# RHnejad/3D_PoseEstimation

Measured on AMD Instinct MI355X. Metric: poses/sec fwd+bwd, 17-joint lifting batch 4096; MPJPE vs ref, higher is better.
Workload: dtype f16x3 (two fp16 planes per fp32 operand, 3 fp16 MFMAs per product, fp32 accumulate); 1 GPU; BASELINE configs[1]: phase1_lifting LinearModel 34-1024-2x(1024-1024)-51, BN+ReLU+Dropout(0.5), one train_1.py step = zero_grad+forward+MSE+backward+AdamW; launch=eager (one call per kernel), per_gpu_batch=4096, global_batch=4096, parallelism=dp1

## Files before the change

### 3d_poseestimation_amd/_lib.py

```python
import ctypes
import os

import torch

_HERE = os.path.dirname(os.path.abspath(__file__))
LIB_PATH = os.environ.get("POSELIFT_LIB") or os.path.join(_HERE, "csrc", "libposelift.so")

PL_F32, PL_BF16, PL_BF16X6, PL_F16X3 = 0, 1, 2, 3


GATHER_FN = ctypes.CFUNCTYPE(ctypes.c_int, ctypes.c_void_p, ctypes.c_void_p, ctypes.c_int64, ctypes.c_void_p)


class PLSync(ctypes.Structure):
    _fields_ = [("world", ctypes.c_int32), ("rank", ctypes.c_int32), ("gather", GATHER_FN),
                ("user", ctypes.c_void_p)]


class PLL1Term(ctypes.Structure):
    _fields_ = [("a", ctypes.c_void_p), ("b", ctypes.c_void_p), ("n", ctypes.c_int64),
                ("da", ctypes.c_void_p), ("db", ctypes.c_void_p)]


L1_MAX_TERMS = 8


class PLDesc(ctypes.Structure):
    _fields_ = [
        ("in_dim", ctypes.c_int32), ("hidden", ctypes.c_int32), ("out_dim", ctypes.c_int32),
        ("num_stage", ctypes.c_int32), ("bn", ctypes.c_int32), ("dtype", ctypes.c_int32),
        ("p_dropout", ctypes.c_float), ("bn_eps", ctypes.c_float), ("bn_momentum", ctypes.c_float),
        ("reserved", ctypes.c_int32),
        ("params", ctypes.c_void_p), ("bn_running", ctypes.c_void_p), ("bn_batches", ctypes.c_void_p),
        ("sync", ctypes.POINTER(PLSync)),
        ("step_dev", ctypes.c_void_p),
        ("wplanes", ctypes.c_void_p), ("wplanes_valid", ctypes.c_int32), ("reserved2", ctypes.c_int32),
    ]


ADAMW_MAX_SEGS = 8


class PLAdamWSeg(ctypes.Structure):
    _fields_ = [("offset", ctypes.c_int64), ("numel", ctypes.c_int64), ("h", ctypes.c_void_p), ("l", ctypes.c_void_p)]


class PLAdamWPlanes(ctypes.Structure):
    _fields_ = [("nseg", ctypes.c_int32), ("kind", ctypes.c_int32), ("scale", ctypes.c_float),
                ("reserved", ctypes.c_int32), ("seg", PLAdamWSeg * ADAMW_MAX_SEGS)]


class PLAdamWStep(ctypes.Structure):
    _fields_ = [("m", ctypes.c_void_p), ("v", ctypes.c_void_p), ("lr", ctypes.c_float), ("lr_dev", ctypes.c_void_p),
                ("beta1", ctypes.c_float), ("beta2", ctypes.c_float), ("eps", ctypes.c_float), ("weight_decay", ctypes.c_float),
                ("t", ctypes.c_int64), ("t_dev", ctypes.c_void_p)]


class PLPlanesEpilogue(ctypes.Structure):
    _fields_ = [("bias", ctypes.c_void_p), ("scale", ctypes.c_void_p), ("shift", ctypes.c_void_p), ("resid", ctypes.c_void_p),
                ("relu", ctypes.c_int32), ("reserved", ctypes.c_int32), ("y_planes", ctypes.c_void_p)]


_c = ctypes
_P = ctypes.c_void_p
_D = ctypes.POINTER(PLDesc)
SIGNATURES = {
    "pl_version": (_c.c_int, []),
    "pl_last_error": (_c.c_char_p, []),
    "pl_num_hidden": (_c.c_int64, [_D]),
    "pl_param_tensors": (_c.c_int64, [_D]),
    "pl_param_offset": (_c.c_int64, [_D, _c.c_int64]),
    "pl_param_numel": (_c.c_int64, [_D, _c.c_int64]),
    "pl_param_arena_floats": (_c.c_int64, [_D]),
    "pl_workspace_bytes": (_c.c_size_t, [_D, _c.c_int64]),
    "pl_workspace_view": (_c.c_int, [_D, _c.c_int64, _c.c_int, _c.c_int64,
                                     _c.POINTER(_c.c_size_t), _c.POINTER(_c.c_size_t)]),
    "pl_workspace_bitmap_format": (_c.c_int, [_D, _c.c_int64, _c.c_int64]),
    "pl_lifter_fwd_eval": (_c.c_int, [_D, _P, _P, _c.c_int64, _P, _c.c_size_t, _P]),
    "pl_lifter_fwd_train": (_c.c_int, [_D, _P, _P, _c.c_int64, _P, _c.c_size_t, _c.c_uint64,
                                       _c.c_uint64, _P, _P]),
    "pl_lifter_bwd": (_c.c_int, [_D, _P, _P, _c.c_int64, _P, _c.c_size_t, _P, _P, _P]),
    "pl_lifter_fwd_eval_saved": (_c.c_int, [_D, _P, _P, _c.c_int64, _P, _c.c_size_t, _P]),
    "pl_lifter_bwd_eval": (_c.c_int, [_D, _P, _P, _c.c_int64, _P, _c.c_size_t, _P, _P, _P]),
    "pl_lifter_bwd_layers": (_c.c_int, [_D, _P, _P, _c.c_int64, _P, _c.c_size_t, _P, _P, _c.c_int, _c.c_int, _P]),
    "pl_lifter_train_fwd_bwd": (_c.c_int, [_D, _P, _P, _c.c_int64, _P, _c.c_size_t, _c.c_uint64, _c.c_uint64,
                                           _P, _P, _P, _c.c_int, _c.c_int, _P]),
    "pl_lifter_step_carries_adamw": (_c.c_int, [_D, _c.c_int64]),
    "pl_lifter_train_step": (_c.c_int, [_D, _P, _P, _c.c_int64, _P, _c.c_size_t, _c.c_uint64, _c.c_uint64,
                                        _P, _P, _P, _c.POINTER(PLAdamWStep), _P]),
    "pl_mse_scratch_bytes": (_c.c_size_t, [_c.c_int64]),
    "pl_mse_fwd_bwd": (_c.c_int, [_P, _P, _c.c_int64, _c.c_float, _P, _P, _P, _P]),
    "pl_l1_scratch_bytes": (_c.c_size_t, [_c.c_int]),
    "pl_l1_terms_fwd_bwd": (_c.c_int, [_c.POINTER(PLL1Term), _c.c_int, _c.c_float, _P, _P, _P]),
    "pl_mpjpe_scratch_bytes": (_c.c_size_t, [_c.c_int64, _c.c_int64]),
    "pl_mpjpe_accum": (_c.c_int, [_P, _P, _c.c_int64, _c.c_int64, _P, _P, _P]),
    "pl_adamw_flat": (_c.c_int, [_P, _P, _P, _P, _c.c_int64, _c.c_float, _c.c_float, _c.c_float,
                                 _c.c_float, _c.c_float, _c.c_int64, _c.c_float, _P]),
    "pl_adamw_flat_dev": (_c.c_int, [_P, _P, _P, _P, _c.c_int64, _P, _c.c_float, _c.c_float, _c.c_float,
                                     _c.c_float, _c.c_int64, _P, _c.c_float, _P]),
    "pl_adamw_flat_planes": (_c.c_int, [_P, _P, _P, _P, _c.c_int64, _c.c_float, _P, _c.c_float, _c.c_float, _c.c_float,
                                        _c.c_float, _c.c_int64, _P, _c.c_float, _c.POINTER(PLAdamWPlanes), _P]),
    "pl_wplanes_bytes": (_c.c_size_t, [_D]),
    "pl_wplanes_layer_bytes": (_c.c_size_t, [_D]),
    "pl_weight_plane_scale": (_c.c_float, []),
    "pl_wplanes_refresh": (_c.c_int, [_D, _P]),
    "pl_flip_pose": (_c.c_int, [_P, _P, _c.c_int64, _c.c_int64, _c.c_int64, _P]),
    "pl_counter_add": (_c.c_int, [_P, _c.c_int64, _P]),
    "pl_flip_pose_ex": (_c.c_int, [_P, _P, _P, _c.c_int64, _c.c_int64, _c.c_int64, _c.c_float, _c.c_float, _P]),
    "pl_flip_w_nhwc": (_c.c_int, [_P, _P, _c.c_int64, _c.c_int64, _c.c_int64, _c.c_int64, _P]),
    "pl_softargmax3d_nhwc_fwd": (_c.c_int, [_P, _c.c_int64, _c.c_int64, _c.c_int64, _c.c_int64, _P, _P, _P]),
    "pl_softargmax3d_nhwc_bwd": (_c.c_int, [_P, _P, _P, _c.c_int64, _c.c_int64, _c.c_int64, _c.c_int64, _P, _P]),
    "pl_conv2d_nhwc_scratch_bytes": (_c.c_size_t, [_c.c_int64, _c.c_int64, _c.c_int64, _c.c_int64, _c.c_int64,
                                                  _c.c_int, _c.c_int, _c.c_int, _c.c_int]),
    "pl_conv2d_nhwc_scratch_bytes_ex": (_c.c_size_t, [_c.c_int64, _c.c_int64, _c.c_int64, _c.c_int64, _c.c_int64,
                                                     _c.c_int, _c.c_int, _c.c_int, _c.c_int, _c.c_int, _c.c_int, _c.c_int]),
    "pl_conv2d_nhwc_fwd": (_c.c_int, [_P, _c.c_int64, _c.c_int64, _c.c_int64, _c.c_int64, _P, _c.c_int64, _c.c_int,
                                      _c.c_int, _c.c_int, _c.c_int, _P, _P, _P, _c.c_int, _P, _P, _c.c_int, _P, _c.c_size_t,
                                      _P]),
    "pl_conv2d_nhwc_wgrad_scratch_bytes": (_c.c_size_t, [_c.c_int64, _c.c_int64, _c.c_int64, _c.c_int64, _c.c_int64,
                                                        _c.c_int, _c.c_int, _c.c_int, _c.c_int]),
    "pl_conv2d_nhwc_wgrad": (_c.c_int, [_P, _c.c_int64, _c.c_int64, _c.c_int64, _c.c_int64, _P, _c.c_int64, _c.c_int,
                                        _c.c_int, _c.c_int, _c.c_int, _P, _c.c_int, _P, _c.c_size_t, _P]),
    "pl_bn_train_scratch_bytes": (_c.c_size_t, [_c.c_int64, _c.c_int64]),
    "pl_bn_train_fwd": (_c.c_int, [_P, _c.c_int64, _c.c_int64, _P, _P, _c.c_float, _c.c_float, _P, _P, _P, _c.c_int,
                                   _P, _P, _P, _P, _P, _P]),
    "pl_bn_train_bwd": (_c.c_int, [_P, _P, _P, _P, _P, _P, _c.c_int64, _c.c_int64, _P, _P, _P, _P, _P]),
    "pl_add_relu_fwd": (_c.c_int, [_P, _P, _c.c_int64, _c.c_int64, _P, _P, _P]),
    "pl_mask_by_bits": (_c.c_int, [_P, _P, _c.c_int64, _c.c_int64, _P, _P]),
    "pl_conv_act_plane_scale": (_c.c_float, []),
    "pl_planes_split": (_c.c_int, [_P, _c.c_int64, _c.c_int, _c.c_float, _P, _P]),
    "pl_planes_split_strided": (_c.c_int, [_P, _P, _P, _c.c_int, _c.c_float, _P, _P]),
    "pl_bn_train_fwd_ex": (_c.c_int, [_P, _c.c_int64, _c.c_int64, _P, _P, _c.c_float, _c.c_float, _P, _P, _P, _c.c_int,
                                      _P, _P, _P, _P, _P, _P, _c.c_int, _P, _P, _P]),
    "pl_gemm_stat_groups": (_c.c_int, [_c.c_int64]),
    "pl_bn_train_bwd_ex": (_c.c_int, [_P, _P, _P, _P, _P, _P, _c.c_int64, _c.c_int64, _P, _P, _P, _P, _P, _c.c_int, _P, _P]),
    "pl_add_relu_fwd_ex": (_c.c_int, [_P, _P, _c.c_int64, _c.c_int64, _P, _P, _P, _c.c_int, _P]),
    "pl_mask_add_by_bits": (_c.c_int, [_P, _P, _P, _c.c_int64, _c.c_int64, _P, _P]),
    "pl_bn_join_bwd": (_c.c_int, [_P, _P, _P, _P, _P, _P, _P, _c.c_int64, _c.c_int64, _P, _P, _P, _P, _P, _P, _c.c_int, _P, _P]),
    "pl_maxpool3x3s2_nhwc": (_c.c_int, [_P, _c.c_int64, _c.c_int64, _c.c_int64, _c.c_int64, _P, _P]),
    "pl_maxpool3x3s2_nhwc_bwd": (_c.c_int, [_P, _P, _c.c_int64, _c.c_int64, _c.c_int64, _c.c_int64, _P, _P]),
    "pl_maxpool3x3s2_nhwc_idx": (_c.c_int, [_P, _c.c_int64, _c.c_int64, _c.c_int64, _c.c_int64, _P, _P, _P]),
    "pl_maxpool3x3s2_nhwc_bwd_idx": (_c.c_int, [_P, _P, _c.c_int64, _c.c_int64, _c.c_int64, _c.c_int64, _P, _P]),
    "pl_upsample2x_zero_nhwc": (_c.c_int, [_P, _c.c_int64, _c.c_int64, _c.c_int64, _c.c_int64, _P, _P]),
    "pl_colsum_scratch_bytes": (_c.c_size_t, [_c.c_int64, _c.c_int64]),
    "pl_colsum": (_c.c_int, [_P, _c.c_int64, _c.c_int64, _P, _P, _P]),
    "pl_deconv4x4s2_nhwc_scratch_bytes": (_c.c_size_t, [_c.c_int64, _c.c_int64, _c.c_int64, _c.c_int64]),
    "pl_deconv4x4s2_nhwc_fwd": (_c.c_int, [_P, _c.c_int64, _c.c_int64, _c.c_int64, _c.c_int64, _P, _c.c_int64, _P, _P,
                                           _c.c_int, _P, _c.c_int, _P, _c.c_size_t, _P]),
    "pl_nhwc_to_nchw": (_c.c_int, [_P, _c.c_int64, _c.c_int64, _c.c_int64, _P, _P]),
    "pl_gather_rows2": (_c.c_int, [_P, _c.c_int64, _P, _c.c_int64, _P, _c.c_int64, _c.c_int64, _P, _P, _P]),
    "pl_flip_tta_pack": (_c.c_int, [_P, _P, _c.c_int64, _c.c_int64, _c.c_int64, _P]),
    "pl_flip_tta_merge": (_c.c_int, [_P, _P, _c.c_int64, _c.c_int64, _c.c_int64, _P]),
    "pl_softargmax_dl_scale": (_c.c_int, [_P, _c.c_int64, _c.c_int, _P, _P]),
    "pl_softargmax_fwd": (_c.c_int, [_P, _c.c_int64, _c.c_int64, _c.c_int64, _c.c_int64, _c.c_int, _c.c_int, _P, _P, _P]),
    "pl_softargmax_bwd": (_c.c_int, [_P, _P, _P, _c.c_int64, _c.c_int64, _c.c_int64, _c.c_int64, _c.c_int, _c.c_int,
                                     _P, _P]),
    "pl_gemm_f32": (_c.c_int, [_c.c_int, _P, _P, _P, _c.c_int64, _c.c_int64, _c.c_int64, _P,
                               _c.c_int, _P, _P]),
    "pl_gemm_arith": (_c.c_int, [_c.c_int, _c.c_int, _P, _P, _P, _c.c_int64, _c.c_int64, _c.c_int64, _P,
                                 _c.c_int, _P, _P]),
    "pl_gemm_planes_scratch_bytes": (_c.c_size_t, [_c.c_int64, _c.c_int64, _c.c_int64]),
    "pl_gemm_planes": (_c.c_int, [_c.c_int, _c.c_int, _P, _P, _P, _c.c_int64, _c.c_int64, _c.c_int64, _P,
                                  _c.c_float, _c.c_float, _P, _P]),
    "pl_gemm_planes_splits": (_c.c_int, [_c.c_int64, _c.c_int64, _c.c_int64]),
    "pl_gemm_planes_raw": (_c.c_int, [_c.c_int, _c.c_int, _P, _c.c_int64, _c.c_int64, _P, _c.c_int64, _c.c_int64, _P,
                                      _c.c_int64, _c.c_int64, _c.c_int64, _P, _c.c_float, _P, _P, _P, _P]),
    "pl_conv2d_planes_fwd": (_c.c_int, [_c.c_int, _P, _c.c_int64, _c.c_int64, _c.c_int64, _c.c_int64, _c.c_int64, _P,
                                        _c.c_int64, _c.c_int64, _c.c_int, _c.c_int, _c.c_int, _c.c_int, _P, _c.c_float, _P, _P, _P]),
    "pl_softargmax3d_nhwc_bwd_ex": (_c.c_int, [_P, _P, _P, _c.c_int64, _c.c_int64, _c.c_int64, _c.c_int64, _P, _P, _c.c_int,
                                               _P, _P]),
# ... 118 lines not shown
```

### 3d_poseestimation_amd/csrc/api.hip

```cpp
#include <stdarg.h>
#include <stdio.h>
#include <stdlib.h>

#include <vector>

#include "adamw.h"
#include "pl_internal.h"

namespace pl {

static thread_local char g_err[512] = "";

void set_error(const char* fmt, ...) {
  va_list ap;
  va_start(ap, fmt);
  vsnprintf(g_err, sizeof(g_err), fmt, ap);
  va_end(ap);
}

namespace {

inline int64_t align_up(int64_t v, int64_t a) { return (v + a - 1) / a * a; }

int check_desc(const PLDesc* d, bool need_arenas) {
// ... 47 lines not shown

struct ParamLayout {
  int L;
  std::vector<int64_t> off, numel;
  int64_t total;
};

ParamLayout param_layout(const PLDesc* d) {
  ParamLayout p;
  p.L = 1 + 2 * d->num_stage;
  int64_t o = 0;
  auto add = [&](int64_t n) {
    p.off.push_back(o);
    p.numel.push_back(n);
    o = align_up(o + n, 64);
  };
  for (int l = 0; l < p.L; ++l) {
    const int64_t fan_in = l == 0 ? d->in_dim : d->hidden;
    add((int64_t)d->hidden * fan_in);
    add(d->hidden);
    add(d->hidden);
    add(d->hidden);
  }
  add((int64_t)d->out_dim * d->hidden);
  add(d->out_dim);
  p.total = o;
  return p;
}

int out_splits(int M, int N, int K) {
  const int tiles = ((M + 127) / 128) * ((N + 127) / 128);
  int s = 256 / tiles;
  const int kmax = K / 128;
  if (s > kmax) s = kmax;
  return s < 1 ? 1 : s;
}

enum class Lin : uint8_t {
  Skinny, Planes, Gemm,
  PlanesMid,
  F32Mid,
};
enum class Stats : uint8_t {
  None,
  InLayer,
  Small,
  InApply,
  Finalize,
};
enum class Bwd : uint8_t {
  PlanesPair, F32Pair,
  SmallLayer, SmallLayerDw,
  InAbove,
  First,
};
struct LayerRoute {
  Lin lin;
  Stats stats;
  Bwd bwd;
  int groups;
  bool bnr_fused;
};
enum class Loss : uint8_t { SmallMse, FromSlabs, PartialOnly };

struct Ws {
  int L, G, RC;
  std::vector<size_t> z, act, bits, mean, rstd, dbpart;
  size_t stat, scale, shift, coef, ga, gb, dz, slabs, outpart, dyout, mse, total;
  size_t act_bytes, bits_bytes;
  size_t slab_floats;
  bool planes;
  int pkind;
  std::vector<size_t> actp, wp;
  std::vector<size_t> sactp;
  std::vector<char> act_f32;
  size_t dzp, amax, dzscale;
  size_t skp_out, skp_in;
  std::vector<size_t> wslab;
  std::vector<LayerRoute> layer;
  bool bn_small;
  bool small_layer;
  bool top_fused;
  bool adam_rides;
  bool small_f16;
  bool eval_small;
  bool out_narrow;
  bool out_skinny;
  Loss loss;
};

Ws plan(const PLDesc* d, int64_t B) {
  Ws w;
  w.L = 1 + 2 * d->num_stage;
  const int H = d->hidden;
  w.G = gemm_stat_groups((int)B);
  w.RC = bwd_row_chunks((int)B, H);
  size_t o = 0;
  auto take = [&](size_t bytes) {
    const size_t at = o;
    o = (size_t)align_up((int64_t)(o + bytes), 256);
    return at;
  };
  w.act_bytes = (size_t)B * H * sizeof(float);
  w.bits_bytes = std::max((size_t)B * bitmap_words_per_row(H), (size_t)H) * sizeof(uint64_t);
  w.pkind = planes_kind(d, B);
  w.planes = w.pkind != 0;
  for (int l = 0; l < w.L; ++l) {
    const bool f32 = !w.planes || (l % 2 == 0) || l == w.L - 1;
    w.act_f32.push_back(f32 ? 1 : 0);
    w.z.push_back(take(w.act_bytes));
    w.act.push_back(f32 ? take(w.act_bytes) : 0);
    w.bits.push_back(take(w.bits_bytes));
    w.mean.push_back(take((size_t)H * 4));
    w.rstd.push_back(take((size_t)H * 4));
    w.dbpart.push_back(take((size_t)w.RC * H * 4));
  }
  const int Pmax = std::max(std::max(w.G, skinny_stat_groups((int)B)), w.RC);
  const size_t amax_pairs = std::max((size_t)((H + 255) / 256) * w.RC, (size_t)(B / 64 + 1) * (H / 32 + 1));
  w.stat = take((size_t)sync_world(d) * ((size_t)2 * Pmax * H + 2 * amax_pairs) * 4);
  w.scale = take((size_t)w.L * H * 4);
  w.shift = take((size_t)w.L * H * 4);
  w.coef = take((size_t)3 * H * 4);
  w.ga = take(w.act_bytes);
  w.gb = take(w.act_bytes);
  w.dz = take(w.act_bytes);
  size_t slab = 0;
  auto need = [&](int M, int N) {
    const int s = tn_splits(M, N, (int)B);
    if (s > 1) slab = std::max(slab, (size_t)s * M * N * 4);
  };
  need(H, d->in_dim);
  need(H, H);
  need(d->out_dim, H);
  {
    const int so = out_splits((int)B, d->out_dim, H);
    if (so > 1) slab = std::max(slab, (size_t)so * B * d->out_dim * 4);
    slab = std::max(slab, (size_t)skinny_chunks((int)B) * std::max(d->in_dim, d->out_dim) * H * 4);
    slab = std::max(slab, skinny_narrow_out_part_floats((int)B, H) * 4);
    if (B <= kThinGemmMaxM && B % 128) slab = std::max(slab, thin_gemm_scratch_floats((int)B, H, H) * 4);
    if (B <= kThinGemmMaxM) slab = std::max(slab, (size_t)(H / 16 + 1) * B * 64 * 4);
  }
  w.slab_floats = slab / 4;
  w.slabs = take(slab);
  w.outpart = take((size_t)std::max(colsum_chunks((int)B), skinny_in_chunks((int)B)) * d->out_dim * 4);
  w.dyout = take((size_t)B * d->out_dim * 4);
  w.mse = take(std::max(pl_mse_scratch_bytes(B * d->out_dim), (size_t)256));
  w.dzp = w.amax = w.dzscale = 0;
  w.skp_out = take((size_t)skinny_in_chunks((int)B) * d->out_dim * H * 4);
  w.skp_in = take((size_t)skinny_in_chunks((int)B) * d->in_dim * H * 4);
  if (w.planes) {
    w.wslab.push_back(0);
    for (int l = 1; l < w.L; ++l) w.wslab.push_back(take((size_t)tn_splits(H, H, (int)B) * H * H * 4));
    for (int l = 0; l + 1 < w.L; ++l) w.actp.push_back(take(w.act_bytes));
    w.wp.push_back(0);
    for (int l = 1; l < w.L; ++l) w.wp.push_back(take((size_t)H * H * 4));
    w.dzp = take(w.act_bytes);
    w.amax = take(std::max((size_t)((H + 255) / 256) * w.RC, (size_t)(B / 64) * (H / 32)) * 2 * 4);
    w.dzscale = take((size_t)w.L * 2 * 4);
  }
  if (d->dtype == PL_F16X3 && B <= kThinGemmMaxM)
    for (int l = 0; l + 1 < w.L; ++l) w.sactp.push_back(take(w.act_bytes));
  w.total = o;

  const int world = sync_world(d);
  const bool first_ok = small_first_ok(d->in_dim), mid_ok = B * world <= 512 && small_layer_ok(2, H, H);
  w.bn_small = d->bn && !w.planes && world == 1 && B >= 2 && B <= kBnSmallRows;
  w.small_layer = w.bn_small && small_layer_ok((int)B, H, H);
  w.top_fused = w.small_layer && small_top_ok(d->out_dim);
  const bool small_head = w.top_fused && (d->num_stage > 0 || first_ok);
  w.adam_rides = small_head && H % 128 == 0;
  w.small_f16 = d->dtype == PL_F16X3 && !w.sactp.empty() && first_ok;
  w.eval_small = d->bn && B <= kThinGemmMaxM && small_layer_ok(2, H, H) && first_ok && small_top_ok(d->out_dim);
  w.out_narrow = skinny_narrow_out_supported(H, d->out_dim);
  w.out_skinny = skinny_supported(d->out_dim, H);
  const int so = w.out_narrow ? skinny_narrow_out_splits((int)B, H) : 0;
  w.loss = small_head ? Loss::SmallMse : (so && mse_from_slabs_supported(so, d->out_dim)) ? Loss::FromSlabs : Loss::PartialOnly;
  for (int l = 0; l < w.L; ++l) {
    LayerRoute r;
    if (l == 0) r.lin = skinny_supported(d->in_dim, H) ? Lin::Skinny : Lin::Gemm;
    else if (w.planes) r.lin = w.pkind == 2 && mid_ok ? Lin::PlanesMid : Lin::Planes;
    else r.lin = d->bn && d->dtype != PL_BF16 && B > kBnSmallRows && mid_ok ? Lin::F32Mid : Lin::Gemm;
    r.groups = r.lin == Lin::Skinny ? skinny_stat_groups((int)B) : w.G;
    const bool tile = w.small_layer && (l > 0 || first_ok);
    if (!d->bn) r.stats = Stats::None;
    else if (w.bn_small) r.stats = tile ? Stats::InLayer : Stats::Small;
    else r.stats = world == 1 && r.groups >= 1 && r.groups <= 4 ? Stats::InApply : Stats::Finalize;
    if (l == 0) r.bwd = tile && w.L > 1 ? Bwd::InAbove : Bwd::First;
    else if (!w.small_layer) r.bwd = w.planes ? Bwd::PlanesPair : Bwd::F32Pair;
    else r.bwd = H % 128 == 0 ? Bwd::SmallLayerDw : Bwd::SmallLayer;
    r.bnr_fused = w.planes && (l < w.L - 1 || w.out_skinny);
    w.layer.push_back(r);
  }
  return w;
}

struct BnrSlab {
  float *mine, *amax_mine, *amax0;
  int64_t floats_per_rank;
  int world;
};
BnrSlab bnr_slab(const PLDesc* d, const Ws& w, void* ws, int rc, int n_amax, bool eval_bn) {
  BnrSlab b;
  float* stat = reinterpret_cast<float*>(static_cast<char*>(ws) + w.stat);
  b.world = eval_bn ? 1 : sync_world(d);
  const int64_t sums = (int64_t)2 * rc * d->hidden;
  if (b.world == 1) {
    b.mine = stat;
    b.amax_mine = b.amax0 = w.amax ? reinterpret_cast<float*>(static_cast<char*>(ws) + w.amax) : nullptr;
    b.floats_per_rank = sums;
    return b;
  }
  b.floats_per_rank = sums + 2 * (int64_t)n_amax;
  b.mine = stat + (size_t)sync_rank(d) * b.floats_per_rank;
  b.amax_mine = b.mine + sums;
  b.amax0 = stat + sums;
  return b;
}

struct Layer {
  const float *W, *b, *gamma, *beta;
  float *gW, *gb, *ggamma, *gbeta;
  float *rm, *rv;
  int64_t* nbt;
  int K;
};

Layer layer_of(const PLDesc* d, const ParamLayout& pl_, float* grads, int l) {
  Layer y;
  const int H = d->hidden;
  y.K = l == 0 ? d->in_dim : H;
  y.W = d->params + pl_.off[4 * l];
  y.b = d->params + pl_.off[4 * l + 1];
  y.gamma = d->params + pl_.off[4 * l + 2];
  y.beta = d->params + pl_.off[4 * l + 3];
  y.gW = grads ? grads + pl_.off[4 * l] : nullptr;
  y.gb = grads ? grads + pl_.off[4 * l + 1] : nullptr;
  y.ggamma = grads ? grads + pl_.off[4 * l + 2] : nullptr;
  y.gbeta = grads ? grads + pl_.off[4 * l + 3] : nullptr;
  y.rm = d->bn_running ? d->bn_running + (size_t)l * 2 * H : nullptr;
  y.rv = d->bn_running ? d->bn_running + (size_t)l * 2 * H + H : nullptr;
  y.nbt = d->bn_batches ? d->bn_batches + l : nullptr;
  return y;
}

inline float* f32(void* ws, size_t off) { return reinterpret_cast<float*>(static_cast<char*>(ws) + off); }
inline uint64_t* u64(void* ws, size_t off) { return reinterpret_cast<uint64_t*>(static_cast<char*>(ws) + off); }

int check_ws(const Ws& w, void* ws, size_t bytes) {
  if (!ws) PL_FAIL(PL_EWORKSPACE, "workspace is NULL");
  if (reinterpret_cast<uintptr_t>(ws) & 255) PL_FAIL(PL_EWORKSPACE, "workspace not 256-byte aligned");
  if (bytes < w.total) PL_FAIL(PL_EWORKSPACE, "workspace too small: %zu < %zu bytes", bytes, w.total);
  return PL_OK;
}

inline unsigned short* u16(void* ws, size_t off) { return reinterpret_cast<unsigned short*>(static_cast<char*>(ws) + off); }
inline const unsigned short* sact_in(const Ws& w, void* ws, int l) { return w.small_f16 && l > 0 ? u16(ws, w.sactp[l - 1]) : nullptr; }
inline unsigned short* sact_out(const Ws& w, void* ws, int l) { return w.small_f16 && l + 1 < w.L ? u16(ws, w.sactp[l]) : nullptr; }

inline unsigned short* wplane(const PLDesc* d, const Ws& w, void* ws, int l) {
  if (d->wplanes) {
    const size_t per = (size_t)d->hidden * d->hidden * 2 * (w.pkind == 2 ? 2 : 1);
    return reinterpret_cast<unsigned short*>(static_cast<char*>(d->wplanes) + (size_t)(l - 1) * per);
  }
  return u16(ws, w.wp[l]);
}

int split_weight_planes(const PLDesc* d, const ParamLayout& P, const Ws& w, void* ws, hipStream_t s) {
  if (d->wplanes && d->wplanes_valid) return PL_OK;
  if (d->wplanes && (reinterpret_cast<uintptr_t>(d->wplanes) & 15)) PL_FAIL(PL_EINVAL, "wplanes not 16-byte aligned");
  const int64_t n = (int64_t)d->hidden * d->hidden;
  for (int l = 1; l < w.L; ++l) {
    unsigned short* q = wplane(d, w, ws, l);
    PlaneOut po = {q, q + n, kWeightPlaneScale, nullptr, w.pkind};
    PL_TRY(launch_split_planes(d->params + P.off[4 * l], n, po, s));
  }
  return PL_OK;
}

PlanesGemmArgs planes_args(int pkind, const unsigned short* A, int64_t a_plane, int lda, const unsigned short* Bm,
                           int64_t b_plane, int ldb, float* C, int M, int N, int K, float out_scale,
                           const float* dyn_inv) {
  PlanesGemmArgs g = {};
  g.A = A; g.B = Bm; g.a_plane = a_plane; g.b_plane = b_plane; g.lda = lda; g.ldb = ldb;
  g.mode = pkind == 2 ? 2 : 0;
  g.out_scale = pkind == 2 ? out_scale : 1.0f;
  g.dyn_inv = pkind == 2 ? dyn_inv : nullptr;
  g.e.C = C; g.e.M = M; g.e.N = N; g.e.K = K; g.e.ldc = N; g.e.split_k = 1;
  return g;
}

int gemm_out_layer(bool narrow, const float* h, const float* W, const float* bias, float* y, int M, int N, int K,
                   float* slabs, hipStream_t s) {
  if (narrow) return launch_skinny_narrow_out(h, W, bias, y, M, K, N, slabs, s);
  GemmArgs g = {};
  g.A = h; g.B = W; g.M = M; g.N = N; g.K = K; g.lda = K; g.ldb = K; g.ldc = N;
  const int splits = out_splits(M, N, K);
  if (splits > 1) {
    g.C = slabs; g.split_k = splits;
    PL_TRY(launch_gemm_f32(kNT, g, s));
    return launch_reduce_slabs_bias(slabs, splits, M, N, bias, y, s);
  }
  g.C = y; g.bias = bias; g.split_k = 1;
  return launch_gemm_f32(kNT, g, s);
}

int gemm_tn_reduced(const float* A, int lda, const float* Bm, int ldb, float* C, int M, int N, int K,
                    float* slabs, hipStream_t s) {
  GemmArgs g = {};
  g.A = A; g.B = Bm; g.M = M; g.N = N; g.K = K; g.lda = lda; g.ldb = ldb; g.ldc = N;
  const int splits = tn_splits(M, N, K);
  if (splits > 1) {
    g.C = slabs; g.split_k = splits;
    PL_TRY(launch_gemm_f32(kTN, g, s));
    return launch_reduce_slabs(slabs, splits, (int64_t)M * N, C, s);
  }
  g.C = C; g.split_k = 1;
  return launch_gemm_f32(kTN, g, s);
}

}
}

using namespace pl;

extern "C" int pl_version(void) { return PL_VERSION; }
extern "C" const char* pl_last_error(void) { return g_err; }

extern "C" int64_t pl_num_hidden(const PLDesc* d) { return d ? 1 + 2 * (int64_t)d->num_stage : PL_EINVAL; }
extern "C" int64_t pl_param_tensors(const PLDesc* d) { return d ? 4 * (1 + 2 * (int64_t)d->num_stage) + 2 : PL_EINVAL; }
extern "C" int64_t pl_param_offset(const PLDesc* d, int64_t i) {
  if (check_desc(d, false) != PL_OK) return PL_EINVAL;
  const ParamLayout p = param_layout(d);
  if (i < 0 || i >= (int64_t)p.off.size()) { set_error("tensor index %lld out of range", (long long)i); return PL_EINVAL; }
  return p.off[i];
}
extern "C" int64_t pl_param_numel(const PLDesc* d, int64_t i) {
  if (check_desc(d, false) != PL_OK) return PL_EINVAL;
  const ParamLayout p = param_layout(d);
  if (i < 0 || i >= (int64_t)p.numel.size()) { set_error("tensor index %lld out of range", (long long)i); return PL_EINVAL; }
  return p.numel[i];
}
extern "C" int64_t pl_param_arena_floats(const PLDesc* d) {
  if (check_desc(d, false) != PL_OK) return PL_EINVAL;
  return param_layout(d).total;
}

extern "C" size_t pl_wplanes_layer_bytes(const PLDesc* d) {
// ... 160 lines not shown
                                    slabs_here ? d->params + P.off[4 * w.L] : nullptr, slabs_here ? f32(ws, w.slabs) : nullptr,
                                    d->out_dim, sact_in(w, ws, l), sact_out(w, ws, l)));
      a_in = f32(ws, w.act[l]);
      continue;
    }
    if (st == Stats::InApply || st == Stats::Finalize) {
      g.stat_sum = stat + (size_t)sync_rank(d) * 2 * r.groups * H;
      g.stat_m2 = g.stat_sum + (size_t)r.groups * H;
    }
    if (r.lin == Lin::Skinny) {
      PL_TRY(launch_skinny_wide_out(a_in, ly.W, ly.b, g.C, (int)B, ly.K, H, false, g.stat_sum, g.stat_m2, s));
    } else if (r.lin == Lin::PlanesMid) {
      PL_TRY(launch_small_linear_stats(nullptr, u16(ws, w.actp[l - 1]), ly.W, ly.b, g.C, (int)B, H, H, g.stat_sum, g.stat_m2, r.groups, s));
    } else if (r.lin == Lin::Planes) {
      PlanesGemmArgs pg = planes_args(w.pkind, u16(ws, w.actp[l - 1]), BH, H, wplane(d, w, ws, l), (int64_t)H * H, H, g.C, (int)B, H, H,
                                      1.0f / (kActPlaneScale * kWeightPlaneScale), nullptr);
      pg.e.bias = ly.b; pg.e.stat_sum = g.stat_sum; pg.e.stat_m2 = g.stat_m2;
      PL_TRY(launch_gemm_planes(kNT, pg, s));
    } else if (r.lin == Lin::F32Mid) {
      PL_TRY(launch_small_linear_stats(a_in, nullptr, ly.W, ly.b, g.C, (int)B, H, H, g.stat_sum, g.stat_m2, r.groups, s));
    } else {
      PL_TRY(launch_gemm_f32(kNT, g, s));
    }
    const float *scale = nullptr, *shift = nullptr;
    BnFinalizeArgs fin = {};
    float* sc = f32(ws, w.scale) + (size_t)l * H;
    float* sh = f32(ws, w.shift) + (size_t)l * H;
    if (d->bn && eval_bn) {
      PL_TRY(launch_bn_eval_stats(ly.gamma, ly.beta, ly.rm, ly.rv, d->bn_eps, H, f32(ws, w.mean[l]), f32(ws, w.rstd[l]),
                                  sc, sh, s));
      scale = sc; shift = sh;
    } else if (st == Stats::InApply) {
      fin = BnFinalizeArgs{stat, r.groups, 64, ly.gamma, ly.beta, d->bn_eps, d->bn_momentum, ly.rm, ly.rv, ly.nbt,
                           f32(ws, w.mean[l]), f32(ws, w.rstd[l])};
    } else if (st == Stats::Finalize) {
      PL_TRY(sync_gather(d, stat, (int64_t)2 * r.groups * H, s));
      PL_TRY(launch_bn_finalize(stat, r.groups, sync_world(d), (int)B, H, ly.gamma, ly.beta, d->bn_eps,
                                d->bn_momentum, ly.rm, ly.rv, ly.nbt, f32(ws, w.mean[l]),
                                f32(ws, w.rstd[l]), sc, sh, s));
      scale = sc; shift = sh;
    } else if (st == Stats::Small) {
      PL_TRY(launch_bn_small_fwd(g.C, ly.gamma, ly.beta, d->bn_eps, d->bn_momentum, ly.rm, ly.rv, ly.nbt, f32(ws, w.mean[l]),
                                 f32(ws, w.rstd[l]), resid, f32(ws, w.act[l]), u64(ws, w.bits[l]), (int)B, H, d->p_dropout, seed,
                                 step, l, inject_keep ? inject_keep + (size_t)l * inj_stride : nullptr, s, d->step_dev));
      a_in = f32(ws, w.act[l]);
      continue;
    }
    PlaneOut po = {nullptr, nullptr, kActPlaneScale, nullptr, 0};
    if (w.planes && l + 1 < w.L) { po.h = u16(ws, w.actp[l]); po.l = po.h + BH; po.kind = w.pkind; }
    float* act = w.act_f32[l] ? f32(ws, w.act[l]) : nullptr;
    PL_TRY(launch_bn_apply(g.C, scale, shift, resid, act, u64(ws, w.bits[l]), (int)B, H,
                           eval_bn ? 0.f : d->p_dropout, seed, step, l,
                           inject_keep ? inject_keep + (size_t)l * inj_stride : nullptr, s, &po,
                           eval_bn ? nullptr : d->step_dev, st == Stats::InApply ? &fin : nullptr));
    a_in = act;
  }
  if (head_slabs) return PL_OK;
  if (defer_out_reduce)
    return launch_skinny_narrow_out(a_in, d->params + P.off[4 * w.L], d->params + P.off[4 * w.L + 1], y, (int)B, H, d->out_dim,
                                    f32(ws, w.slabs), s, false);
  return gemm_out_layer(w.out_narrow, a_in, d->params + P.off[4 * w.L], d->params + P.off[4 * w.L + 1], y, (int)B,
                        d->out_dim, H, f32(ws, w.slabs), s);
}

static int bwd_impl(const PLDesc* d, const float* x, const float* dy, int64_t B, void* ws, size_t ws_bytes,
                    float* dx, float* grads, void* stream, bool do_output, int l_hi, int l_lo, bool eval_bn = false,
                    float* loss_out = nullptr, int loss_partials = 0, const PLAdamWStep* adam = nullptr) {
  PL_TRY(check_desc(d, true));
  if (!x || !dy || !grads) PL_FAIL(PL_EINVAL, "pl_lifter_bwd: null x/dy/flat_grads");
  if (B <= 0) PL_FAIL(PL_ESHAPE, "pl_lifter_bwd: B=%lld", (long long)B);
  const Ws w = plan(d, B);
  PL_TRY(check_ws(w, ws, ws_bytes));
  const ParamLayout P = param_layout(d);
  hipStream_t s = (hipStream_t)stream;
  const int H = d->hidden, O = d->out_dim, Bi = (int)B;
  const float kscale = (!eval_bn && d->p_dropout > 0.f && d->p_dropout < 1.f) ? 1.0f / (1.0f - d->p_dropout) : 1.0f;
  float* slabs = f32(ws, w.slabs);
  float* GA = f32(ws, w.ga);
  float* GB = f32(ws, w.gb);
  float* DZ = f32(ws, w.dz);
  const int64_t BH = B * H;
  const int n_amax = ((H + 255) / 256) * w.RC;
  std::vector<const float*> jpart; std::vector<float*> jout; std::vector<int> jR, jH, jkind, jtrans;
  auto job = [&](const float* part, float* out, int R, int Hj, int kind, int transK) {
    jpart.push_back(part); jout.push_back(out); jR.push_back(R); jH.push_back(Hj); jkind.push_back(kind); jtrans.push_back(transK);
  };

  const bool small = !eval_bn && w.bn_small, sl = !eval_bn && w.small_layer;
  auto bn_layer = [&](int l) {
    const Layer y = layer_of(d, P, grads, l);
    SmallBnLayer b = {f32(ws, w.z[l]), f32(ws, w.mean[l]), f32(ws, w.rstd[l]), y.gamma, u64(ws, w.bits[l]),
                      w.layer[l].stats != Stats::InLayer, y.ggamma, y.gbeta, y.gb};
    return b;
  };
  const int n_loss_part = loss_partials > 0 ? loss_partials : mse_partials(B * O);
  const bool top_fused = do_output && !eval_bn && w.top_fused && l_hi == w.L - 1 && l_hi >= l_lo;
  const bool adam_rides = adam && top_fused && l_lo == 0 && w.adam_rides;
  auto ride = [&](int64_t lo, int64_t hi) {
    AdamWRide r = {};
    r.p = const_cast<float*>(d->params) + lo; r.g = grads + lo; r.m = adam->m + lo; r.v = adam->v + lo; r.n = hi - lo;
    r.lr = adam->lr; r.beta1 = adam->beta1; r.beta2 = adam->beta2; r.eps = adam->eps; r.wd = adam->weight_decay; r.gscale = 1.0f;
    r.t = adam->t; r.lr_dev = adam->lr_dev; r.t_dev = adam->t_dev;
    return r;
  };
  if (top_fused) {
    PL_TRY(launch_small_top_bwd(dy, d->params + P.off[4 * w.L], f32(ws, w.act[w.L - 1]), Bi, H, O, GA, grads + P.off[4 * w.L],
                                grads + P.off[4 * w.L + 1], bn_layer(w.L - 1), kscale, DZ, s, f32(ws, w.mse),
                                n_loss_part, 1.0f / (float)(B * O), loss_out, const_cast<uint64_t*>(d->step_dev)));
  } else if (do_output && w.out_skinny) {
    PL_TRY(launch_skinny_wide_in(dy, f32(ws, w.act[w.L - 1]), grads + P.off[4 * w.L], Bi, O, H, false, f32(ws, w.skp_out), s,
                                 false, f32(ws, w.outpart)));
    job(f32(ws, w.skp_out), grads + P.off[4 * w.L], skinny_in_chunks(Bi), O * H, 0, 0);
    job(f32(ws, w.outpart), grads + P.off[4 * w.L + 1], skinny_in_chunks(Bi), O, 0, 0);
    GemmArgs be = {};
    const int lt = w.L - 1;
    if (!eval_bn && w.layer[lt].bnr_fused) {
      const BnrSlab sl = bnr_slab(d, w, ws, Bi / 64, (w.pkind == 2 && lt > 0) ? (Bi / 64) * (H / 32) : 0, eval_bn);
      be.bnr_z = f32(ws, w.z[lt]); be.bnr_bits = u64(ws, w.bits[lt]);
      be.bnr_mean = f32(ws, w.mean[lt]); be.bnr_rstd = f32(ws, w.rstd[lt]); be.bnr_kscale = kscale;
      be.bnr_part_dy = sl.mine; be.bnr_part_dyz = sl.mine + (size_t)(Bi / 64) * H;
      be.bnr_amax = (w.pkind == 2 && lt > 0) ? sl.amax_mine : nullptr;
    }
    PL_TRY(launch_skinny_wide_out(dy, d->params + P.off[4 * w.L], nullptr, GA, Bi, O, H, true, nullptr, nullptr, s, &be));
  } else if (do_output) {
    PL_TRY(gemm_tn_reduced(dy, O, f32(ws, w.act[w.L - 1]), H, grads + P.off[4 * w.L], O, H, Bi, slabs, s));
    PL_TRY(launch_colsum_partial(dy, Bi, O, f32(ws, w.outpart), s));
    job(f32(ws, w.outpart), grads + P.off[4 * w.L + 1], colsum_chunks(Bi), O, 0, 0);
    GemmArgs g = {};
    g.A = dy; g.B = d->params + P.off[4 * w.L]; g.C = GA; g.M = Bi; g.N = H; g.K = O; g.lda = O; g.ldb = H; g.ldc = H;
    g.split_k = 1;
    PL_TRY(launch_gemm_f32(kNN, g, s));
  }

  for (int l = l_hi; l >= l_lo; --l) {
    const Layer ly = layer_of(d, P, grads, l);
    const LayerRoute& r = w.layer[l];
    const float* gin = (l % 2 == 1) ? GB : GA;
    const uint64_t* bits = u64(ws, w.bits[l]);
    const float* z = f32(ws, w.z[l]);
    const bool pl_layer = r.bwd == Bwd::PlanesPair;
    float* dzs = (pl_layer && w.pkind == 2) ? f32(ws, w.dzscale) + 2 * l : nullptr;
    PlaneOut dzo = {nullptr, nullptr, 1.0f, dzs, 0};
    if (pl_layer) { dzo.h = u16(ws, w.dzp); dzo.l = dzo.h + BH; dzo.kind = w.pkind; }
    auto dzbuf = [&](int layer) { return (sl && (layer & 1)) ? GB : DZ; };
    float* DZl = dzbuf(l);
    if (sl && (l < l_hi || top_fused)) {
    } else if (small) {
      PL_TRY(launch_bn_small_bwd(gin, bits, z, f32(ws, w.mean[l]), f32(ws, w.rstd[l]), ly.gamma, kscale, Bi, H, DZl, ly.ggamma,
                                 ly.gbeta, ly.gb, s, r.stats == Stats::InLayer));
    } else if (d->bn) {
      const bool fr = !eval_bn && r.bnr_fused;
      const int rc_l = fr ? Bi / 64 : w.RC;
      const int n_amax_l = fr ? (Bi / 64) * (l == w.L - 1 ? H / 32 : H / 64) : n_amax;
      const BnrSlab sl = bnr_slab(d, w, ws, rc_l, dzs ? n_amax_l : 0, eval_bn);
      float* stat = f32(ws, w.stat);
      if (!fr)
        PL_TRY(launch_bn_bwd_reduce(gin, bits, z, f32(ws, w.mean[l]), f32(ws, w.rstd[l]), kscale, Bi, H,
                                    sl.mine, sl.mine + (size_t)rc_l * H, s, 0, dzs ? sl.amax_mine : nullptr, rc_l));
      if (!eval_bn) PL_TRY(sync_gather(d, stat, sl.floats_per_rank, s));
      PL_TRY(launch_bn_bwd_finalize(stat, rc_l, eval_bn ? 1 : sync_world(d), eval_bn ? 0 : sync_rank(d), Bi, H, ly.gamma,
                                    f32(ws, w.rstd[l]), f32(ws, w.coef), ly.ggamma, ly.gbeta, s,
                                    dzs ? sl.amax0 : nullptr, n_amax_l, dzs, eval_bn ? 1 : 0, sl.floats_per_rank, sl.world));
    } else {
      PL_TRY(launch_fill(ly.ggamma, H, 0.f, s));
      PL_TRY(launch_fill(ly.gbeta, H, 0.f, s));
    }
    if (!small) {
      PL_TRY(launch_bn_bwd_dz(gin, bits, z, f32(ws, w.mean[l]), f32(ws, w.rstd[l]), f32(ws, w.coef), kscale,
                              d->bn, Bi, H, pl_layer ? nullptr : DZ, f32(ws, w.dbpart[l]), s, 0, &dzo, w.RC));
      job(f32(ws, w.dbpart[l]), ly.gb, w.RC, H, 0, 0);
    }
    const float* a_in = l == 0 ? x : (w.planes ? nullptr : f32(ws, w.act[l - 1]));
    if (pl_layer) {
      const int splits = tn_splits(H, H, Bi);
      PlanesGemmArgs nn = planes_args(w.pkind, u16(ws, w.dzp), BH, H, wplane(d, w, ws, l), (int64_t)H * H, H,
                                      (l % 2 == 1) ? GA : GB, Bi, H, H, 1.0f / kWeightPlaneScale, dzs ? dzs + 1 : nullptr);
      if (l % 2 == 1) nn.e.addend = GA;
      if (!eval_bn && w.layer[l - 1].bnr_fused) {
        const bool lower_scaled = w.pkind == 2 && l - 1 > 0;
        const BnrSlab sl = bnr_slab(d, w, ws, Bi / 64, lower_scaled ? (Bi / 64) * (H / 64) : 0, eval_bn);
        nn.e.bnr_z = f32(ws, w.z[l - 1]);
        nn.e.bnr_bits = u64(ws, w.bits[l - 1]);
        nn.e.bnr_mean = f32(ws, w.mean[l - 1]);
        nn.e.bnr_rstd = f32(ws, w.rstd[l - 1]);
        nn.e.bnr_kscale = kscale;
        nn.e.bnr_part_dy = sl.mine;
        nn.e.bnr_part_dyz = sl.mine + (size_t)(Bi / 64) * H;
        nn.e.bnr_amax = lower_scaled ? sl.amax_mine : nullptr;
      }
      float* wsl = f32(ws, w.wslab[l]);
      PlanesGemmArgs tn = planes_args(w.pkind, u16(ws, w.dzp), BH, H, u16(ws, w.actp[l - 1]), BH, H,
                                      splits > 1 ? wsl : ly.gW, H, H, Bi, 1.0f / kActPlaneScale, dzs ? dzs + 1 : nullptr);
      tn.e.split_k = splits;
      PL_TRY(launch_gemm_planes_pair(nn, tn, s));
      if (splits > 1) job(wsl, ly.gW, splits, H * H, 1, 0);
    } else if (l > 0) {
      GemmArgs g = {};
      g.A = DZl; g.B = ly.W; g.M = Bi; g.N = H; g.K = H; g.lda = H; g.ldb = H; g.ldc = H; g.split_k = 1;
      if (l % 2 == 1) { g.C = GA; g.addend = GA; } else { g.C = GB; }
      g.arith = arith_of(d);
      g.thin_scratch = slabs; g.thin_scratch_floats = w.slab_floats;
      GemmArgs t = {};
      t.arith = g.arith;
      t.A = DZl; t.B = a_in; t.M = H; t.N = H; t.K = Bi; t.lda = H; t.ldb = H; t.ldc = H; t.split_k = 1; t.C = ly.gW;
      if (sl && (r.bwd == Bwd::SmallLayer || r.bwd == Bwd::SmallLayerDw)) {
        const bool dw_rides = r.bwd == Bwd::SmallLayerDw;
        if (l - 1 >= l_lo) {
          const bool w1 = l == 1 && w.layer[0].bwd == Bwd::InAbove;
          AdamWRide ar = {};
          if (adam_rides) ar = ride(P.off[4 * l + 1], l == w.L - 1 ? P.total : P.off[4 * (l + 1) + 1]);
          PL_TRY(launch_small_layer_bwd(DZl, ly.W, (l % 2 == 1) ? GA : nullptr, (l % 2 == 1) ? GA : nullptr, Bi, H, H,
                                        bn_layer(l - 1), kscale, dzbuf(l - 1), s, dw_rides ? a_in : nullptr,
                                        dw_rides ? ly.gW : nullptr, w1 ? x : nullptr, w1 ? grads + P.off[0] : nullptr, d->in_dim,
                                        adam_rides ? &ar : nullptr));
          if (dw_rides) continue;
        } else {
          PL_TRY(launch_gemm_f32(kNN, g, s));
        }
        PL_TRY(launch_gemm_f32(kTN, t, s));
        continue;
      }
      const int splits = tn_splits(H, H, Bi);
      t.split_k = splits; t.C = splits > 1 ? slabs : ly.gW;
      PL_TRY(launch_gemm_f32_pair(g, t, s));
      if (splits > 1) PL_TRY(launch_reduce_slabs(slabs, splits, (int64_t)H * H, ly.gW, s));
    } else if (r.bwd == Bwd::InAbove && sl && l_hi > 0) {
    } else if (r.lin == Lin::Skinny) {
      PL_TRY(launch_skinny_wide_in(a_in, DZ, ly.gW, Bi, ly.K, H, true, f32(ws, w.skp_in), s, false));
      job(f32(ws, w.skp_in), ly.gW, skinny_in_chunks(Bi), ly.K * H, 0, ly.K);
    } else {
      PL_TRY(gemm_tn_reduced(DZ, H, a_in, ly.K, ly.gW, H, ly.K, Bi, slabs, s));
    }
    if (l == 0 && dx) {
      GemmArgs g = {};
      g.A = DZ; g.B = ly.W; g.C = dx; g.M = Bi; g.N = d->in_dim; g.K = H; g.lda = H; g.ldb = d->in_dim;
      g.ldc = d->in_dim; g.split_k = 1;
      PL_TRY(launch_gemm_f32(kNN, g, s));
    }
  }
  float inv_n = 0.f;
  uint64_t* tick = nullptr;
  if (loss_out && !top_fused) {
    const int64_t n = B * O;
    job(f32(ws, w.mse), loss_out, n_loss_part, 1, 2, 0);
    inv_n = 1.0f / (float)n;
    tick = const_cast<uint64_t*>(d->step_dev);
  }
  if (!jpart.empty())
    PL_TRY(launch_reduce_rows_multi(jpart.data(), jR.data(), jH.data(), jout.data(), (int)jpart.size(), s, jkind.data(),
                                    jtrans.data(), inv_n, tick));
  if (adam) {
    const int64_t n = adam_rides ? (w.L > 1 ? P.off[4 * 1 + 1] : P.total) : P.total;
    float* p = const_cast<float*>(d->params);
    if (adam->lr_dev)
      PL_TRY(pl_adamw_flat_dev(p, grads, adam->m, adam->v, n, adam->lr_dev, adam->beta1, adam->beta2, adam->eps,
                               adam->weight_decay, adam->t, adam->t_dev, 1.0f, stream));
    else
      PL_TRY(pl_adamw_flat(p, grads, adam->m, adam->v, n, adam->lr, adam->beta1, adam->beta2, adam->eps, adam->weight_decay,
                           adam->t, 1.0f, stream));
  }
  return PL_OK;
}

extern "C" int pl_lifter_bwd(const PLDesc* d, const float* x, const float* dy, int64_t B, void* ws,
                             size_t ws_bytes, float* dx, float* grads, void* stream) {
  if (!d) PL_FAIL(PL_EINVAL, "descriptor is NULL");
  return bwd_impl(d, x, dy, B, ws, ws_bytes, dx, grads, stream, true, 2 * d->num_stage, 0);
}

extern "C" int pl_lifter_bwd_eval(const PLDesc* d, const float* x, const float* dy, int64_t B, void* ws,
                                  size_t ws_bytes, float* dx, float* grads, void* stream) {
  if (!d) PL_FAIL(PL_EINVAL, "descriptor is NULL");
  return bwd_impl(d, x, dy, B, ws, ws_bytes, dx, grads, stream, true, 2 * d->num_stage, 0, true);
}

static int check_range(const PLDesc* d, int hi, int lo, const char* who) {
  const int L = 1 + 2 * d->num_stage;
  if (lo < 0 || hi < lo || hi > L) PL_FAIL(PL_EINVAL, "%s: layer range hi=%d lo=%d outside 0..%d", who, hi, lo, L);
  return PL_OK;
}

extern "C" int pl_lifter_bwd_layers(const PLDesc* d, const float* x, const float* dy, int64_t B, void* ws,
                                    size_t ws_bytes, float* dx, float* grads, int hi, int lo, void* stream) {
  PL_TRY(check_desc(d, true));
  PL_TRY(check_range(d, hi, lo, "pl_lifter_bwd_layers"));
  const int L = 1 + 2 * d->num_stage;
  return bwd_impl(d, x, dy, B, ws, ws_bytes, lo == 0 ? dx : nullptr, grads, stream, hi == L, hi == L ? L - 1 : hi, lo);
}

extern "C" int pl_gemm_f32(int layout, const float* A, const float* Bm, float* C, int64_t M, int64_t N,
                           int64_t K, const float* bias, int split_k, float* slabs, void* stream) {
  return pl_gemm_arith(layout, PL_F32, A, Bm, C, M, N, K, bias, split_k, slabs, stream);
}

extern "C" int pl_gemm_arith(int layout, int arith, const float* A, const float* Bm, float* C, int64_t M,
                             int64_t N, int64_t K, const float* bias, int split_k, float* slabs, void* stream) {
  if (layout < 0 || layout > 2) PL_FAIL(PL_EINVAL, "pl_gemm_f32: layout %d", layout);
  if ((arith < 0 || arith > 2) && arith != 5 && arith != 6) PL_FAIL(PL_EDTYPE, "pl_gemm_arith: arith %d", arith);
  if (M <= 0 || N <= 0 || K <= 0 || M > INT32_MAX || N > INT32_MAX || K > INT32_MAX)
    PL_FAIL(PL_ESHAPE, "pl_gemm_f32: bad shape");
  GemmArgs g = {};
  g.A = A; g.B = Bm; g.C = C; g.M = (int)M; g.N = (int)N; g.K = (int)K; g.bias = bias;
  g.lda = layout == kTN ? (int)M : (int)K;
  g.ldb = layout == kNT ? (int)K : (int)N;
  g.ldc = (int)N;
  g.split_k = 1;
  g.arith = arith;
  hipStream_t s = (hipStream_t)stream;
  if (split_k > 1) {
    if (layout != kTN || !slabs || bias) PL_FAIL(PL_EINVAL, "pl_gemm_f32: split_k needs layout 2, slabs and no bias");
    g.C = slabs; g.split_k = split_k;
    PL_TRY(launch_gemm_f32(kTN, g, s));
    return launch_reduce_slabs(slabs, split_k, M * N, C, s);
  }
  return launch_gemm_f32((GemmLayout)layout, g, s);
}

static void set_planes_mode(PlanesGemmArgs& g, int mode, float out_scale, const float* dyn_inv) {
  g.mode = mode == PL_F16X3 ? 2 : 0;
  g.out_scale = mode == PL_F16X3 ? out_scale : 1.0f;
  g.dyn_inv = mode == PL_F16X3 ? dyn_inv : nullptr;
}

extern "C" size_t pl_gemm_planes_scratch_bytes(int64_t M, int64_t N, int64_t K) {
  if (M <= 0 || N <= 0 || K <= 0) return 0;
  return (size_t)(align_up(M * K * 4, 256) + align_up(N * K * 4, 256));
}

extern "C" int pl_gemm_planes(int layout, int mode, const float* A, const float* Bm, float* C, int64_t M, int64_t N,
                              int64_t K, const float* bias, float scale_a, float scale_b, void* scratch, void* stream) {
// ... 141 lines not shown
static int deconv_planes_fwd(const char* who, int mode, const void* x_planes, int64_t x_plane, int64_t B, int64_t H, int64_t W,
                             int64_t Cin, const void* wsub_planes, int64_t wsub_plane, int64_t Cout, float* y, float out_scale,
                             const float* dyn_inv, const PLPlanesEpilogue* ep, void* stream) {
  if (mode != PL_F16X3 && mode != PL_BF16) PL_FAIL(PL_EDTYPE, "%s: mode %d", who, mode);
  if (!x_planes || !wsub_planes || (!y && !(ep && ep->y_planes)) || Cout <= 0) PL_FAIL(PL_EINVAL, "%s: null pointer", who);
  if (B <= 0 || H <= 0 || W <= 0 || Cin <= 0 || B * H * W > INT32_MAX) PL_FAIL(PL_ESHAPE, "%s: bad geometry", who);
  if (ep && ep->resid) PL_FAIL(PL_EINVAL, "%s: no residual on a transposed convolution", who);
  const int64_t K = 4 * Cin, nsub = Cout * K;
  for (int ph = 0; ph < 2; ++ph)
    for (int pw = 0; pw < 2; ++pw) {
      PlanesGemmArgs g = {};
      g.e.conv_cin = (int)Cin; g.e.conv_h = (int)H; g.e.conv_w = (int)W; g.e.conv_ho = (int)H; g.e.conv_wo = (int)W;
      g.e.conv_kw = 2; g.e.conv_stride = 1;
      g.e.conv_pad_h = ph ? 0 : 1; g.e.conv_pad_w = pw ? 0 : 1;
      g.e.scat_on = 1; g.e.scat_ph = ph; g.e.scat_pw = pw;
      g.A = static_cast<const unsigned short*>(x_planes);
      g.B = static_cast<const unsigned short*>(wsub_planes) + (size_t)(ph * 2 + pw) * nsub;
      g.a_plane = x_plane; g.b_plane = wsub_plane; g.lda = 0; g.ldb = (int)K;
      set_planes_mode(g, mode, out_scale, dyn_inv);
      g.e.C = y; g.e.M = (int)(B * H * W); g.e.N = (int)Cout; g.e.K = (int)K; g.e.ldc = (int)Cout; g.e.split_k = 1;
      PL_TRY(apply_planes_epilogue(g.e, mode, ep, B * 4 * H * W * Cout, who));
      PL_TRY(launch_gemm_planes(kNT, g, (hipStream_t)stream));
    }
  return PL_OK;
}

extern "C" int pl_deconv4x4s2_planes_fwd_ep(int mode, const void* x_planes, int64_t x_plane, int64_t B, int64_t H, int64_t W,
                                            int64_t Cin, const void* wsub_planes, int64_t wsub_plane, int64_t Cout, float* y,
                                            float out_scale, const PLPlanesEpilogue* ep, void* stream) {
  return deconv_planes_fwd("pl_deconv4x4s2_planes_fwd_ep", mode, x_planes, x_plane, B, H, W, Cin, wsub_planes, wsub_plane, Cout, y,
                           out_scale, nullptr, ep, stream);
}

extern "C" int pl_deconv4x4s2_planes_fwd(int mode, const void* x_planes, int64_t x_plane, int64_t B, int64_t H, int64_t W,
                                         int64_t Cin, const void* wsub_planes, int64_t wsub_plane, int64_t Cout, float* y,
                                         float out_scale, const float* dyn_inv, void* stream) {
  return deconv_planes_fwd("pl_deconv4x4s2_planes_fwd", mode, x_planes, x_plane, B, H, W, Cin, wsub_planes, wsub_plane, Cout, y,
                           out_scale, dyn_inv, nullptr, stream);
}

extern "C" int pl_conv2d_planes_wgrad(int mode, const void* dz_planes, int64_t dz_plane, const void* x_planes, int64_t x_plane,
                                      int64_t B, int64_t H, int64_t W, int64_t Cin, int64_t Cout, int KH, int KW, int stride,
                                      int pad, float* dw, float out_scale, const float* dyn_inv, float* slabs, void* stream) {
  return pl_conv2d_planes_wgrad_hw(mode, dz_planes, dz_plane, x_planes, x_plane, B, H, W, Cin, Cout, KH, KW, stride, stride, pad,
                                   pad, pad, dw, out_scale, dyn_inv, slabs, stream);
}

extern "C" int pl_conv2d_planes_wgrad_hw(int mode, const void* dz_planes, int64_t dz_plane, const void* x_planes,
                                         int64_t x_plane, int64_t B, int64_t H, int64_t W, int64_t Cin, int64_t Cout, int KH,
                                         int KW, int stride_h, int stride_w, int pad_h, int pad_w, int pad_w_right, float* dw,
                                         float out_scale, const float* dyn_inv, float* slabs, void* stream) {
  if (mode != PL_F16X3 && mode != PL_BF16) PL_FAIL(PL_EDTYPE, "pl_conv2d_planes_wgrad: mode %d", mode);
  if (!dz_planes || !x_planes || !dw || Cout <= 0) PL_FAIL(PL_EINVAL, "pl_conv2d_planes_wgrad: null pointer");
  PlanesGemmArgs g = {};
  int64_t Ho, Wo;
  PL_TRY(conv_planes_geom(g.e, B, H, W, Cin, KH, KW, stride_h, pad_h, &Ho, &Wo, "pl_conv2d_planes_wgrad", stride_w, pad_w, pad_w_right));
  const int64_t N = (int64_t)KH * KW * Cin, K = B * Ho * Wo;
  g.A = static_cast<const unsigned short*>(dz_planes); g.B = static_cast<const unsigned short*>(x_planes);
  g.a_plane = dz_plane; g.b_plane = x_plane; g.lda = (int)Cout; g.ldb = 0;
  set_planes_mode(g, mode, out_scale, dyn_inv);
  g.e.M = (int)Cout; g.e.N = (int)N; g.e.K = (int)K; g.e.ldc = (int)N;
  return launch_planes_split_k("pl_conv2d_planes_wgrad", kTN, g, dw, slabs, (hipStream_t)stream);
}

extern "C" int pl_prof_enable(int on) { return prof_enable(on); }
extern "C" int pl_prof_read(double min_flops, double max_flops, double* ms_total, int64_t* launches,
                            double* flops_total) {
  if (!ms_total || !launches || !flops_total) PL_FAIL(PL_EINVAL, "pl_prof_read: null pointer");
  return prof_read(min_flops, max_flops, ms_total, launches, flops_total);
}

static int train_fwd_bwd_impl(const PLDesc* d, const float* x, const float* target, int64_t B, void* ws, size_t ws_bytes,
                              uint64_t seed, uint64_t step, float* y, float* loss, float* grads, int hi, int lo, void* stream,
                              const PLAdamWStep* adam);

extern "C" int pl_lifter_train_fwd_bwd(const PLDesc* d, const float* x, const float* target, int64_t B, void* ws,
                                       size_t ws_bytes, uint64_t seed, uint64_t step, float* y, float* loss,
                                       float* grads, int hi, int lo, void* stream) {
  return train_fwd_bwd_impl(d, x, target, B, ws, ws_bytes, seed, step, y, loss, grads, hi, lo, stream, nullptr);
}

extern "C" int pl_lifter_step_carries_adamw(const PLDesc* d, int64_t B) {
  PL_TRY(check_desc(d, false));
  return B > 0 && plan(d, B).adam_rides ? 1 : 0;
}

extern "C" int pl_lifter_train_step(const PLDesc* d, const float* x, const float* target, int64_t B, void* ws, size_t ws_bytes,
                                    uint64_t seed, uint64_t step, float* y, float* loss, float* grads, const PLAdamWStep* opt,
                                    void* stream) {
  if (!opt || !opt->m || !opt->v || (opt->lr_dev != nullptr) != (opt->t_dev != nullptr) || opt->t < (opt->t_dev ? 0 : 1))
    PL_FAIL(PL_EINVAL, "pl_lifter_train_step: bad optimizer description");
  if (!d) PL_FAIL(PL_EINVAL, "descriptor is NULL");
  return train_fwd_bwd_impl(d, x, target, B, ws, ws_bytes, seed, step, y, loss, grads, 1 + 2 * d->num_stage, 0, stream, opt);
}

static int train_fwd_bwd_impl(const PLDesc* d, const float* x, const float* target, int64_t B, void* ws, size_t ws_bytes,
                              uint64_t seed, uint64_t step, float* y, float* loss, float* grads, int hi, int lo, void* stream,
                              const PLAdamWStep* adam) {
  PL_TRY(check_desc(d, true));
  if (!x || !target || !y || !loss || !grads) PL_FAIL(PL_EINVAL, "pl_lifter_train_fwd_bwd: null pointer");
  if (B <= 0) PL_FAIL(PL_ESHAPE, "pl_lifter_train_fwd_bwd: B=%lld", (long long)B);
  PL_TRY(check_range(d, hi, lo, "pl_lifter_train_fwd_bwd"));
  const Ws w = plan(d, B);
  PL_TRY(check_ws(w, ws, ws_bytes));
  float* dy = f32(ws, w.dyout);
  const int L = 1 + 2 * d->num_stage;
  if (hi == L && w.loss == Loss::PartialOnly) {
    PL_TRY(pl_lifter_fwd_train(d, x, y, B, ws, ws_bytes, seed, step, nullptr, stream));
    PL_TRY(mse_partial_only(y, target, B * d->out_dim, 1.0f, dy, f32(ws, w.mse), stream));
  } else if (hi == L) {
    const int H = d->hidden, O = d->out_dim;
    PL_TRY(fwd_saved_impl(d, x, y, B, ws, ws_bytes, seed, step, nullptr, stream, false, true));
    const float* bias = d->params + param_layout(d).off[4 * L + 1];
    if (w.loss == Loss::SmallMse)
      PL_TRY(launch_small_mse(f32(ws, w.slabs), H / 16, (int)B, O, bias, target, 1.0f, y, dy, f32(ws, w.mse), (hipStream_t)stream));
    else
      PL_TRY(mse_partial_from_slabs(f32(ws, w.slabs), skinny_narrow_out_splits((int)B, H), (int)B, O, bias, target, 1.0f, y, dy,
                                    f32(ws, w.mse), stream));
  }
  return bwd_impl(d, x, dy, B, ws, ws_bytes, nullptr, grads, stream, hi == L, hi == L ? L - 1 : hi, lo, false,
                  hi == L ? loss : nullptr, w.loss == Loss::SmallMse ? small_mse_partials((int)B, d->out_dim) : 0, adam);
}
```

### 3d_poseestimation_amd/csrc/elementwise.hip

```cpp
#include "adamw.h"
#include "bn_pieces.h"
#include "philox.h"
#include <stdlib.h>

#include "pl_internal.h"
#include "plane_store.h"

namespace pl {
namespace {

constexpr int NTHR = 256;

__device__ __forceinline__ float4 ld4(const float* p) { return *reinterpret_cast<const float4*>(p); }
__device__ __forceinline__ void st4(float* p, float4 v) { *reinterpret_cast<float4*>(p) = v; }

__global__ __launch_bounds__(256) void split_planes_kernel(const float* __restrict__ x, int64_t n4, PlaneOut o) {
  const PlaneDst d = plane_dst(o);
  const int64_t stride = (int64_t)gridDim.x * blockDim.x;
  for (int64_t i = (int64_t)blockIdx.x * blockDim.x + threadIdx.x; i < n4; i += stride)
    store_planes4(d, (size_t)i * 4, ld4(x + 4 * i));
}

struct Strided4 { int d1, d2, d3; int64_t s0, s1, s2, s3; };
__global__ __launch_bounds__(256) void split_planes_strided_kernel(const float* __restrict__ x, Strided4 v, int64_t n4, PlaneOut o) {
  const PlaneDst d = plane_dst(o);
  const int64_t stride = (int64_t)gridDim.x * blockDim.x;
  const int q3 = v.d3 >> 2;
  for (int64_t i = (int64_t)blockIdx.x * blockDim.x + threadIdx.x; i < n4; i += stride) {
    const int i3 = (int)(i % q3) * 4;
    int64_t r = i / q3;
    const int i2 = (int)(r % v.d2); r /= v.d2;
    const int i1 = (int)(r % v.d1);
    const int64_t i0 = r / v.d1;
    const float* p = x + i0 * v.s0 + i1 * v.s1 + i2 * v.s2 + (int64_t)i3 * v.s3;
    store_planes4(d, (size_t)i * 4, make_float4(p[0], p[v.s3], p[2 * v.s3], p[3 * v.s3]));
  }
}

constexpr int RCOLS = 16, RPARTS = 16;

__device__ __forceinline__ float parts_sum(float v, float (*red)[RCOLS], int cl, int part) {
  red[part][cl] = v;
  __syncthreads();
  float t = 0.f;
#pragma unroll
  for (int q = 0; q < RPARTS; ++q) t += red[q][cl];
  __syncthreads();
  return t;
}

__device__ __forceinline__ float bn_m2_term(float gsum, float gm2, float fn, float mean) {
#pragma clang fp contract(off)
  const float d = gsum / fn - mean;
  return gm2 + fn * d * d;
}

__global__ __launch_bounds__(NTHR) void bn_finalize_kernel(
    const float* __restrict__ stat, int G, int world, int Br, int H, int gs,
    const float* __restrict__ gamma, const float* __restrict__ beta, float eps, float momentum,
    float* running_mean, float* running_var, int64_t* batches, float* mean_out, float* rstd_out,
    float* scale_out, float* shift_out) {
  __shared__ float red[RPARTS][RCOLS];
  const int cl = threadIdx.x & (RCOLS - 1), part = threadIdx.x / RCOLS;
  const int c = blockIdx.x * RCOLS + cl;
  const bool ok = c < H;
  const int GT = G * world;
  const float Bt = (float)Br * (float)world;
  const size_t GH = (size_t)G * H;
  constexpr int KEEP = 4;
  float ks[KEEP], km[KEEP];
  const bool keep = GT <= KEEP * RPARTS;
#pragma unroll
  for (int q = 0; q < KEEP; ++q) {
    const int g = part + q * RPARTS;
    ks[q] = km[q] = 0.f;
    if (ok && keep && g < GT) {
      const int r = g / G, gl = g - r * G;
      const size_t at = (size_t)r * 2 * GH + (size_t)gl * H + c;
      ks[q] = stat[at]; km[q] = stat[at + GH];
    }
  }
  float ga = 0.f, be = 0.f, rm0 = 0.f, rv0 = 0.f;
  if (part == 0 && ok) {
    ga = gamma[c]; be = beta[c];
    if (running_mean) { rm0 = running_mean[c]; rv0 = running_var[c]; }
  }
// ... 734 lines not shown
  float4 mu = zero, rs = zero, c0 = zero, c1 = zero, c2 = zero;
  if (c < H && bn) {
    const int cc = c % Hc;
    mu = ld4(mean + cc); rs = ld4(rstd + cc);
    c0 = ld4(coef + cc); c1 = ld4(coef + Hc + cc); c2 = ld4(coef + 2 * Hc + cc);
  }
  if (bn) bn_bwd_dz_rows<true>(g, bits, z, mu, rs, c0, c1, c2, kscale, B, H, dz, part_db, pd, sm);
  else bn_bwd_dz_rows<false>(g, bits, z, mu, rs, c0, c1, c2, kscale, B, H, dz, part_db, pd, sm);
}

__global__ void reduce_slabs_kernel(const float* __restrict__ slabs, int nslab, int64_t n,
                                    float* __restrict__ out, int vec) {
  const int64_t stride = (int64_t)gridDim.x * blockDim.x;
  int64_t i = (int64_t)blockIdx.x * blockDim.x + threadIdx.x;
  if (vec) {
    const int64_t n4 = n >> 2;
    for (; i < n4; i += stride) {
      float4 a = ld4(slabs + 4 * i);
      int s = 1;
      for (; s + 4 <= nslab; s += 4) {
        float4 b[4];
#pragma unroll
        for (int u = 0; u < 4; ++u) b[u] = ld4(slabs + (size_t)(s + u) * n + 4 * i);
        __builtin_amdgcn_sched_barrier(0);
#pragma unroll
        for (int u = 0; u < 4; ++u) { a.x += b[u].x; a.y += b[u].y; a.z += b[u].z; a.w += b[u].w; }
      }
      for (; s < nslab; ++s) {
        const float4 b = ld4(slabs + (size_t)s * n + 4 * i);
        a.x += b.x; a.y += b.y; a.z += b.z; a.w += b.w;
      }
      st4(out + 4 * i, a);
    }
  } else {
    for (; i < n; i += stride) {
      float a = slabs[i];
      for (int s = 1; s < nslab; ++s) a += slabs[(size_t)s * n + i];
      out[i] = a;
    }
  }
}

__global__ void reduce_slabs_bias_kernel(const float* __restrict__ slabs, int nslab, int64_t n, int cols,
                                         const float* __restrict__ bias, float* __restrict__ out) {
  const int64_t stride = (int64_t)gridDim.x * blockDim.x;
  for (int64_t i = (int64_t)blockIdx.x * blockDim.x + threadIdx.x; i < n; i += stride) {
    float a = bias ? bias[i % cols] : 0.f;
    for (int s = 0; s < nslab; ++s) a += slabs[(size_t)s * n + i];
    out[i] = a;
  }
}

__global__ __launch_bounds__(NTHR) void colsum_partial_kernel(const float* __restrict__ X, int rows,
                                                              int cols, int rpc, float* __restrict__ part) {
  __shared__ float sm[4][64];
  const int cl = threadIdx.x & 63, rl = threadIdx.x >> 6;
  const int r0 = blockIdx.x * rpc, r1 = min(rows, r0 + rpc);
  for (int c0 = 0; c0 < cols; c0 += 64) {
    const int c = c0 + cl;
    float s = 0.f;
    if (c < cols)
      for (int r = r0 + rl; r < r1; r += 4) s += X[(size_t)r * cols + c];
    sm[rl][cl] = s;
    __syncthreads();
    if (rl == 0 && c < cols) part[(size_t)blockIdx.x * cols + c] = (sm[0][cl] + sm[1][cl]) + (sm[2][cl] + sm[3][cl]);
    __syncthreads();
  }
}

__device__ __forceinline__ float block_sum(float v, float* sm) {
#pragma unroll
  for (int o = 32; o > 0; o >>= 1) v += __shfl_xor(v, o);
  const int lane = threadIdx.x & 63, wave = threadIdx.x >> 6;
  if (lane == 0) sm[wave] = v;
  __syncthreads();
  float t = 0.f;
  const int nw = blockDim.x >> 6;
  for (int w = 0; w < nw; ++w) t += sm[w];
  __syncthreads();
  return t;
}

constexpr int kMaxRowJobs = 16;
struct RowJobs { const float* part[kMaxRowJobs]; float* out[kMaxRowJobs]; int R[kMaxRowJobs]; int H[kMaxRowJobs];
                 int kind[kMaxRowJobs]; int transK[kMaxRowJobs]; float inv_n; uint64_t* tick; };
__global__ __launch_bounds__(NTHR) void reduce_rows_multi_kernel(RowJobs j) {
  __shared__ float red[RPARTS][RCOLS];
  const int job = blockIdx.y;
  const int R = j.R[job], H = j.H[job];
  const float* __restrict__ part = j.part[job];
  if (j.kind[job] == 2) {
    if (blockIdx.x) return;
    float acc = 0.f;
    for (int i = threadIdx.x; i < R; i += blockDim.x) acc += part[i];
    const float t = block_sum(acc, &red[0][0]);
    if (threadIdx.x == 0) {
      j.out[job][0] = t * j.inv_n;
      if (j.tick) j.tick[0] += 1;
    }
    return;
  }
  if (j.kind[job] == 1) {
    const int n4 = H >> 2;
    if (R == 4) {
      for (int i = blockIdx.x * NTHR + threadIdx.x; i < n4; i += gridDim.x * NTHR) {
        const float* __restrict__ q = part + 4 * (size_t)i;
        float4 a = ld4(q);
        const float4 b1 = ld4(q + (size_t)H), b2 = ld4(q + 2 * (size_t)H), b3 = ld4(q + 3 * (size_t)H);
        a.x += b1.x; a.y += b1.y; a.z += b1.z; a.w += b1.w;
        a.x += b2.x; a.y += b2.y; a.z += b2.z; a.w += b2.w;
        a.x += b3.x; a.y += b3.y; a.z += b3.z; a.w += b3.w;
        st4(j.out[job] + 4 * (size_t)i, a);
      }
      return;
    }
    for (int i = blockIdx.x * NTHR + threadIdx.x; i < n4; i += gridDim.x * NTHR) {
      float4 a = ld4(part + 4 * (size_t)i);
      for (int sl = 1; sl < R; ++sl) {
        const float4 b = ld4(part + (size_t)sl * H + 4 * (size_t)i);
        a.x += b.x; a.y += b.y; a.z += b.z; a.w += b.w;
      }
      st4(j.out[job] + 4 * (size_t)i, a);
    }
    return;
  }
  if (blockIdx.x * RCOLS >= H) return;
  const int cl = threadIdx.x & (RCOLS - 1), p = threadIdx.x / RCOLS;
  const int c = blockIdx.x * RCOLS + cl;
  float a = 0.f;
  if (c < H)
#pragma unroll 8
    for (int k = p; k < R; k += RPARTS) a += part[(size_t)k * H + c];
  const float t = parts_sum(a, red, cl, p);
  if (p == 0 && c < H) {
    const int K = j.transK[job];
    if (K > 0) {
      const int Hc = H / K, k = c / Hc, col = c - k * Hc;
      j.out[job][(size_t)col * K + k] = t;
    } else {
      j.out[job][c] = t;
    }
  }
}

__global__ void bn_fold_eval_kernel(const float* __restrict__ bias, const float* __restrict__ gamma,
                                    const float* __restrict__ beta, const float* __restrict__ rm,
                                    const float* __restrict__ rv, float eps, int bn, int H,
                                    float* __restrict__ scale, float* __restrict__ shift) {
  const int c = blockIdx.x * blockDim.x + threadIdx.x;
  if (c >= H) return;
  if (bn) {
    const float s = gamma[c] * (1.0f / sqrtf(rv[c] + eps));
    scale[c] = s;
    shift[c] = fmaf(bias[c] - rm[c], s, beta[c]);
  } else {
    scale[c] = 1.f;
    shift[c] = bias[c];
  }
}

__global__ void bn_eval_stats_kernel(const float* __restrict__ gamma, const float* __restrict__ beta,
                                     const float* __restrict__ rm, const float* __restrict__ rv, float eps, int H,
                                     float* __restrict__ mean, float* __restrict__ rstd, float* __restrict__ scale,
                                     float* __restrict__ shift) {
  const int c = blockIdx.x * blockDim.x + threadIdx.x;
  if (c >= H) return;
  const float r = 1.0f / sqrtf(rv[c] + eps), sc = gamma[c] * r;
  mean[c] = rm[c]; rstd[c] = r; scale[c] = sc; shift[c] = bn_shift_of(beta[c], rm[c], sc);
}

__global__ void fill_kernel(float* p, int64_t n, float v) {
  const int64_t stride = (int64_t)gridDim.x * blockDim.x;
  for (int64_t i = (int64_t)blockIdx.x * blockDim.x + threadIdx.x; i < n; i += stride) p[i] = v;
}

__global__ __launch_bounds__(NTHR) void mse_partial_kernel(const float* __restrict__ pred,
                                                           const float* __restrict__ tgt, int64_t n,
                                                           float coef, float* __restrict__ dpred,
                                                           float* __restrict__ part) {
  __shared__ float sm[4];
  const int64_t stride = (int64_t)gridDim.x * blockDim.x;
  float acc = 0.f;
  for (int64_t i = (int64_t)blockIdx.x * blockDim.x + threadIdx.x; i < n; i += stride) {
    const float d = pred[i] - tgt[i];
    acc = fmaf(d, d, acc);
    if (dpred) dpred[i] = d * coef;
  }
  const float t = block_sum(acc, sm);
  if (threadIdx.x == 0) part[blockIdx.x] = t;
}

template <int NS, int N>
__global__ __launch_bounds__(NTHR) void mse_partial_from_slabs_kernel(const float* __restrict__ part, int B,
                                                                      const float* __restrict__ bias,
                                                                      const float* __restrict__ tgt, float coef,
                                                                      float* __restrict__ y, float* __restrict__ dpred,
                                                                      float* __restrict__ mpart) {
  __shared__ float sm[4];
  const int64_t n = (int64_t)B * N;
  const int64_t stride = (int64_t)gridDim.x * blockDim.x;
  const size_t slab = (size_t)B * 64;
  float acc = 0.f;
  for (int64_t i0 = (int64_t)blockIdx.x * blockDim.x + threadIdx.x; i0 < n; i0 += 4 * stride) {
    float u[4][NS], t[4], bs[4];
    int64_t idx[4];
#pragma unroll
    for (int q = 0; q < 4; ++q) {
      idx[q] = i0 + q * stride;
      const bool ok = idx[q] < n;
      const int r = ok ? (int)(idx[q] / N) : 0, c = ok ? (int)(idx[q] - (int64_t)r * N) : 0;
      const float* p = part + (size_t)r * 64 + c;
#pragma unroll
      for (int s = 0; s < NS; ++s) u[q][s] = ok ? p[(size_t)s * slab] : 0.f;
      t[q] = ok ? tgt[idx[q]] : 0.f;
      bs[q] = (ok && bias) ? bias[c] : 0.f;
    }
#pragma unroll
    for (int q = 0; q < 4; ++q) {
      if (idx[q] >= n) continue;
      float a = bs[q];
#pragma unroll
      for (int s = 0; s < NS; ++s) a += u[q][s];
      y[idx[q]] = a;
      const float d = a - t[q];
      acc = fmaf(d, d, acc);
      dpred[idx[q]] = d * coef;
    }
  }
  const float tsum = block_sum(acc, sm);
  if (threadIdx.x == 0) mpart[blockIdx.x] = tsum;
}

__global__ __launch_bounds__(NTHR) void mse_final_kernel(const float* __restrict__ part, int np,
                                                         float inv_n, float* __restrict__ loss, uint64_t* tick) {
  __shared__ float sm[4];
  float acc = 0.f;
  for (int i = threadIdx.x; i < np; i += blockDim.x) acc += part[i];
  const float t = block_sum(acc, sm);
  if (threadIdx.x == 0) {
    loss[0] = t * inv_n;
    if (tick) tick[0] += 1;
  }
}

constexpr int L1_BLOCKS = 64;
struct L1Terms { PLL1Term t[PL_L1_MAX_TERMS]; };

__global__ __launch_bounds__(NTHR) void l1_partial_kernel(L1Terms T, float grad_scale, float* __restrict__ part) {
  __shared__ float sm[4];
  const PLL1Term q = T.t[blockIdx.y];
  const float coef = grad_scale / (float)q.n;
  float acc = 0.f;
  for (int64_t i = (int64_t)blockIdx.x * NTHR + threadIdx.x; i < q.n; i += (int64_t)L1_BLOCKS * NTHR) {
    const float d = q.a[i] - q.b[i];
    acc += fabsf(d);
    const float g = d > 0.f ? coef : (d < 0.f ? -coef : 0.f);
    if (q.da) q.da[i] = g;
    if (q.db) q.db[i] = -g;
  }
  const float t = block_sum(acc, sm);
  if (threadIdx.x == 0) part[blockIdx.y * L1_BLOCKS + blockIdx.x] = t;
}

__global__ __launch_bounds__(64) void l1_final_kernel(const float* __restrict__ part, L1Terms T,
                                                      float* __restrict__ losses) {
  float v = part[blockIdx.x * L1_BLOCKS + threadIdx.x];
#pragma unroll
  for (int o = 32; o > 0; o >>= 1) v += __shfl_xor(v, o);
  if (threadIdx.x == 0) losses[blockIdx.x] = v / (float)T.t[blockIdx.x].n;
}

__global__ void mpjpe_partial_kernel(const float* __restrict__ pred, const float* __restrict__ tgt,
                                     int B, int J, int rpc, float* __restrict__ part) {
  const int r0 = blockIdx.x * rpc, r1 = min(B, r0 + rpc);
  for (int j = threadIdx.x; j < J; j += blockDim.x) {
    float s = 0.f;
    for (int r = r0; r < r1; ++r) {
      const size_t o = ((size_t)r * J + j) * 3;
      const float dx = pred[o] - tgt[o], dy = pred[o + 1] - tgt[o + 1], dz = pred[o + 2] - tgt[o + 2];
      s += sqrtf(fmaf(dx, dx, fmaf(dy, dy, dz * dz)));
    }
    part[(size_t)blockIdx.x * J + j] = s;
  }
}

__global__ void mpjpe_final_kernel(const float* __restrict__ part, int np, int J,
                                   float* __restrict__ metric) {
  for (int j = threadIdx.x; j < J; j += blockDim.x) {
    float s = 0.f;
    for (int k = 0; k < np; ++k) s += part[(size_t)k * J + j];
    metric[j] += s;
  }
}

__global__ void flip_pose_kernel(const float* __restrict__ in, float* __restrict__ out, int64_t n, int D) {
  const int64_t i = (int64_t)blockIdx.x * blockDim.x + threadIdx.x;
  if (i >= n) return;
  const int d = (int)(i % D);
  const int64_t bj = i / D;
  const int j = (int)(bj % 17);
  const int64_t b = bj / 17;
  const int src = (j >= 1 && j <= 3) ? j + 3 : (j >= 4 && j <= 6) ? j - 3
                : (j >= 11 && j <= 13) ? j + 3 : (j >= 14 && j <= 16) ? j - 3 : j;
  float v = in[(b * 17 + src) * D + d];
  if (d == 0) v = (D == 2) ? 1.0f - v : -v;
  out[i] = v;
}

__device__ __forceinline__ int flip_src_joint(int j) {
  return (j >= 1 && j <= 3) ? j + 3 : (j >= 4 && j <= 6) ? j - 3
       : (j >= 11 && j <= 13) ? j + 3 : (j >= 14 && j <= 16) ? j - 3 : j;
}

// ... 252 lines not shown
}

int launch_bn_bwd_dz(const float* g, const uint64_t* bits, const float* z, const float* mean,
                     const float* rstd, const float* coef, float keep_scale, int bn, int B, int H,
                     float* dz, float* part_db, hipStream_t s, int Hc, const PlaneOut* planes, int rc) {
  dim3 grid((H + 255) / 256, rc > 0 ? rc : bwd_row_chunks(B, H));
  PlaneOut po = planes ? *planes : PlaneOut{nullptr, nullptr, 1.f, nullptr, 0};
  po.nt = (int64_t)B * H * 4 >= kNontemporalBytes ? 1 : 0;
  if (!dz && !po.kind) PL_FAIL(PL_EINVAL, "bn_bwd_dz: nothing to write");
  hipLaunchKernelGGL(bn_bwd_dz_kernel, grid, dim3(NTHR), 0, s, g, bits, z, mean, rstd, coef, keep_scale,
                     bn, B, H, dz, part_db, Hc > 0 ? Hc : H, po);
  PL_CHECK_LAUNCH("bn_bwd_dz");
  return PL_OK;
}

int launch_split_planes(const float* x, int64_t n, const PlaneOut& out, hipStream_t s) {
  if (!x || !out.h || (out.kind == 2 && !out.l) || out.kind < 1 || out.kind > 2) PL_FAIL(PL_EINVAL, "split_planes: bad arguments");
  if ((n & 3) || !aligned16(x) || (reinterpret_cast<uintptr_t>(out.h) & 7) || (reinterpret_cast<uintptr_t>(out.l) & 7))
    PL_FAIL(PL_EINVAL, "split_planes: n %% 4 and alignment");
  const int64_t n4 = n >> 2;
  int blocks = (int)((n4 + 255) / 256);
  if (blocks > 2048) blocks = 2048;
  hipLaunchKernelGGL(split_planes_kernel, dim3(blocks), dim3(256), 0, s, x, n4, out);
  PL_CHECK_LAUNCH("split_planes");
  return PL_OK;
}

int launch_reduce_slabs(const float* slabs, int nslab, int64_t n, float* out, hipStream_t s) {
  if (nslab >= 8 && n <= 65536) {
    hipLaunchKernelGGL(reduce_rows_kernel, dim3(((int)n + RCOLS - 1) / RCOLS), dim3(NTHR), 0, s, slabs, nslab,
                       (int)n, out);
    PL_CHECK_LAUNCH("reduce_rows");
    return PL_OK;
  }
  const int vec = ((n & 3) == 0) && aligned16(slabs) && aligned16(out);
  const int64_t work = vec ? (n >> 2) : n;
  int blocks = (int)((work + NTHR - 1) / NTHR);
  if (blocks > 2048) blocks = 2048;
  if (blocks < 1) blocks = 1;
  hipLaunchKernelGGL(reduce_slabs_kernel, dim3(blocks), dim3(NTHR), 0, s, slabs, nslab, n, out, vec);
  PL_CHECK_LAUNCH("reduce_slabs");
  return PL_OK;
}

int launch_reduce_slabs_bias(const float* slabs, int nslab, int rows, int cols, const float* bias,
                             float* out, hipStream_t s) {
  const int64_t n = (int64_t)rows * cols;
  int blocks = (int)((n + NTHR - 1) / NTHR);
  if (blocks > 2048) blocks = 2048;
  hipLaunchKernelGGL(reduce_slabs_bias_kernel, dim3(blocks), dim3(NTHR), 0, s, slabs, nslab, n, cols, bias, out);
  PL_CHECK_LAUNCH("reduce_slabs_bias");
  return PL_OK;
}

int launch_reduce_rows_multi(const float* const* part, const int* R, const int* H, float* const* out, int njobs,
                             hipStream_t s, const int* kind, const int* transK, float loss_inv_n, uint64_t* loss_tick) {
  for (int base = 0; base < njobs; base += kMaxRowJobs) {
    RowJobs j = {};
    j.inv_n = loss_inv_n; j.tick = loss_tick;
    const int n = njobs - base < kMaxRowJobs ? njobs - base : kMaxRowJobs;
    int gx = 1;
    for (int k = 0; k < n; ++k) {
      j.part[k] = part[base + k]; j.out[k] = out[base + k]; j.R[k] = R[base + k]; j.H[k] = H[base + k];
      j.kind[k] = kind ? kind[base + k] : 0;
      j.transK[k] = transK ? transK[base + k] : 0;
      int need;
      if (j.kind[k] == 1) {
        if ((j.H[k] & 3) || !aligned16(j.part[k]) || !aligned16(j.out[k])) PL_FAIL(PL_EINVAL, "reduce_rows_multi: slab job alignment");
        need = ((j.H[k] >> 2) + NTHR - 1) / NTHR;
        if (need > 1024) need = 1024;
      } else if (j.kind[k] == 2) {
        need = 1;
      } else {
        need = (j.H[k] + RCOLS - 1) / RCOLS;
      }
      if (need > gx) gx = need;
    }
    hipLaunchKernelGGL(reduce_rows_multi_kernel, dim3(gx, n), dim3(NTHR), 0, s, j);
    PL_CHECK_LAUNCH("reduce_rows_multi");
  }
  return PL_OK;
}

int colsum_chunks(int rows) {
  int rc = (rows + 63) / 64;
  if (rc > 64) rc = 64;
  return rc < 1 ? 1 : rc;
}

int launch_colsum_partial(const float* X, int rows, int cols, float* part, hipStream_t s) {
  const int rc = colsum_chunks(rows);
  const int rpc = (rows + rc - 1) / rc;
  hipLaunchKernelGGL(colsum_partial_kernel, dim3(rc), dim3(NTHR), 0, s, X, rows, cols, rpc, part);
  PL_CHECK_LAUNCH("colsum_partial");
  return PL_OK;
}

int launch_bn_fold_eval(const float* bias, const float* gamma, const float* beta, const float* rm,
                        const float* rv, float eps, int bn, int H, float* scale, float* shift,
                        hipStream_t s) {
  hipLaunchKernelGGL(bn_fold_eval_kernel, dim3((H + NTHR - 1) / NTHR), dim3(NTHR), 0, s, bias, gamma, beta,
                     rm, rv, eps, bn, H, scale, shift);
  PL_CHECK_LAUNCH("bn_fold_eval");
  return PL_OK;
}

int launch_bn_eval_stats(const float* gamma, const float* beta, const float* rm, const float* rv, float eps, int H,
                         float* mean, float* rstd, float* scale, float* shift, hipStream_t s) {
  hipLaunchKernelGGL(bn_eval_stats_kernel, dim3((H + NTHR - 1) / NTHR), dim3(NTHR), 0, s, gamma, beta, rm, rv, eps, H,
                     mean, rstd, scale, shift);
  PL_CHECK_LAUNCH("bn_eval_stats");
  return PL_OK;
}

int launch_fill(float* p, int64_t n, float v, hipStream_t s) {
  if (n <= 0) return PL_OK;
  int blocks = (int)((n + NTHR - 1) / NTHR);
  if (blocks > 1024) blocks = 1024;
  hipLaunchKernelGGL(fill_kernel, dim3(blocks), dim3(NTHR), 0, s, p, n, v);
  PL_CHECK_LAUNCH("fill");
  return PL_OK;
}

}

using namespace pl;

static int mse_blocks(int64_t n) {
  int64_t b = (n + NTHR * 4 - 1) / (NTHR * 4);
  if (b > 1024) b = 1024;
  return b < 1 ? 1 : (int)b;
}

extern "C" size_t pl_mse_scratch_bytes(int64_t n) { return (size_t)mse_blocks(n > 0 ? n : 1) * sizeof(float); }

namespace pl {
int mse_fwd_bwd_tick(const float* pred, const float* tgt, int64_t n, float grad_scale, float* dpred, float* loss_out,
                     void* scratch, uint64_t* tick, void* stream);
}

extern "C" int pl_mse_fwd_bwd(const float* pred, const float* tgt, int64_t n, float grad_scale,
                              float* dpred, float* loss_out, void* scratch, void* stream) {
  return mse_fwd_bwd_tick(pred, tgt, n, grad_scale, dpred, loss_out, scratch, nullptr, stream);
}

int pl::mse_partial_only(const float* pred, const float* tgt, int64_t n, float grad_scale, float* dpred, void* scratch,
                         void* stream) {
  if (!pred || !tgt || !scratch) PL_FAIL(PL_EINVAL, "pl_mse_fwd_bwd: null pointer");
  if (n <= 0) PL_FAIL(PL_ESHAPE, "pl_mse_fwd_bwd: n = %lld", (long long)n);
  hipLaunchKernelGGL(mse_partial_kernel, dim3(mse_blocks(n)), dim3(NTHR), 0, (hipStream_t)stream, pred, tgt, n,
                     grad_scale * 2.0f / (float)n, dpred, (float*)scratch);
  PL_CHECK_LAUNCH("mse_partial");
  return PL_OK;
}
int pl::mse_partials(int64_t n) { return mse_blocks(n); }

bool pl::mse_from_slabs_supported(int splits, int N) { return splits == 8 && (N == 51 || N == 34); }
int pl::mse_partial_from_slabs(const float* part, int splits, int B, int N, const float* bias, const float* tgt, float grad_scale,
                               float* y, float* dpred, void* scratch, void* stream) {
  if (!part || !tgt || !y || !dpred || !scratch) PL_FAIL(PL_EINVAL, "mse_partial_from_slabs: null pointer");
  if (!mse_from_slabs_supported(splits, N) || B < 1) PL_FAIL(PL_ESHAPE, "mse_partial_from_slabs: splits=%d N=%d", splits, N);
  const int64_t n = (int64_t)B * N;
  const float coef = grad_scale * 2.0f / (float)n;
  const dim3 grid(mse_blocks(n)), block(NTHR);
  if (N == 51) hipLaunchKernelGGL((mse_partial_from_slabs_kernel<8, 51>), grid, block, 0, (hipStream_t)stream, part, B, bias, tgt, coef, y, dpred, (float*)scratch);
  else hipLaunchKernelGGL((mse_partial_from_slabs_kernel<8, 34>), grid, block, 0, (hipStream_t)stream, part, B, bias, tgt, coef, y, dpred, (float*)scratch);
  PL_CHECK_LAUNCH("mse_partial_from_slabs");
  return PL_OK;
}

int pl::mse_fwd_bwd_tick(const float* pred, const float* tgt, int64_t n, float grad_scale, float* dpred,
                         float* loss_out, void* scratch, uint64_t* tick, void* stream) {
  if (!pred || !tgt || !loss_out || !scratch) PL_FAIL(PL_EINVAL, "pl_mse_fwd_bwd: null pointer");
  if (n <= 0) PL_FAIL(PL_ESHAPE, "pl_mse_fwd_bwd: n = %lld", (long long)n);
  hipStream_t s = (hipStream_t)stream;
  const int nb = mse_blocks(n);
  const float coef = grad_scale * 2.0f / (float)n;
  hipLaunchKernelGGL(mse_partial_kernel, dim3(nb), dim3(NTHR), 0, s, pred, tgt, n, coef, dpred,
                     (float*)scratch);
  PL_CHECK_LAUNCH("mse_partial");
  hipLaunchKernelGGL(mse_final_kernel, dim3(1), dim3(NTHR), 0, s, (const float*)scratch, nb,
                     1.0f / (float)n, loss_out, tick);
  PL_CHECK_LAUNCH("mse_final");
  return PL_OK;
}

static int mpjpe_chunks(int64_t B) {
  int64_t c = (B + 63) / 64;
  if (c > 256) c = 256;
  return c < 1 ? 1 : (int)c;
}

extern "C" size_t pl_mpjpe_scratch_bytes(int64_t B, int64_t joints) {
  return (size_t)mpjpe_chunks(B) * (size_t)(joints > 0 ? joints : 1) * sizeof(float);
}

extern "C" int pl_mpjpe_accum(const float* pred, const float* tgt, int64_t B, int64_t joints,
                              float* metric, void* scratch, void* stream) {
  if (!pred || !tgt || !metric || !scratch) PL_FAIL(PL_EINVAL, "pl_mpjpe_accum: null pointer");
  if (B <= 0 || joints <= 0 || joints > 1024) PL_FAIL(PL_ESHAPE, "pl_mpjpe_accum: B=%lld joints=%lld", (long long)B, (long long)joints);
  hipStream_t s = (hipStream_t)stream;
  const int nc = mpjpe_chunks(B);
  const int rpc = (int)((B + nc - 1) / nc);
  hipLaunchKernelGGL(mpjpe_partial_kernel, dim3(nc), dim3(64), 0, s, pred, tgt, (int)B, (int)joints, rpc,
                     (float*)scratch);
  PL_CHECK_LAUNCH("mpjpe_partial");
  hipLaunchKernelGGL(mpjpe_final_kernel, dim3(1), dim3(64), 0, s, (const float*)scratch, nc, (int)joints,
                     metric);
  PL_CHECK_LAUNCH("mpjpe_final");
  return PL_OK;
}

constexpr int kAdamBlocks = 512;

static int adamw_launch(float* p, const float* g, float* m, float* v, int64_t n, const AdamWIn& in, void* stream) {
  if (!p || !g || !m || !v) PL_FAIL(PL_EINVAL, "pl_adamw_flat: null pointer");
  if (n <= 0 || in.t < (in.t_dev ? 0 : 1)) PL_FAIL(PL_ESHAPE, "pl_adamw_flat: n=%lld t=%lld", (long long)n, (long long)in.t);
  const int vec = aligned16(p) && aligned16(g) && aligned16(m) && aligned16(v);
  int64_t work = vec ? (n >> 2) : n;
  int blocks = (int)((work + NTHR - 1) / NTHR);
  if (blocks > kAdamBlocks) blocks = kAdamBlocks;
  if (blocks < 1) blocks = 1;
  hipLaunchKernelGGL(adamw_kernel, dim3(blocks), dim3(NTHR), 0, (hipStream_t)stream, p, g, m, v, n, in, vec);
  PL_CHECK_LAUNCH("adamw");
  return PL_OK;
}

static AdamWIn adamw_in(float lr, float beta1, float beta2, float eps, float wd, float gscale, int64_t t,
                        const float* lr_dev, const uint64_t* t_dev) {
  AdamWIn in = {};
  in.lr = lr; in.beta1 = beta1; in.beta2 = beta2; in.eps = eps; in.wd = wd; in.gscale = gscale; in.t = t;
  in.lr_dev = lr_dev; in.t_dev = t_dev;
  return in;
}

extern "C" int pl_adamw_flat(float* p, const float* g, float* m, float* v, int64_t n, float lr,
                             float beta1, float beta2, float eps, float weight_decay, int64_t t,
                             float grad_scale, void* stream) {
  return adamw_launch(p, g, m, v, n, adamw_in(lr, beta1, beta2, eps, weight_decay, grad_scale, t, nullptr, nullptr), stream);
}

extern "C" int pl_adamw_flat_dev(float* p, const float* g, float* m, float* v, int64_t n, const float* lr_dev,
                                 float beta1, float beta2, float eps, float weight_decay, int64_t t_base,
                                 const uint64_t* t_dev, float grad_scale, void* stream) {
  if (!lr_dev || !t_dev) PL_FAIL(PL_EINVAL, "pl_adamw_flat_dev: null lr / t pointer");
  return adamw_launch(p, g, m, v, n, adamw_in(0.f, beta1, beta2, eps, weight_decay, grad_scale, t_base, lr_dev, t_dev), stream);
}

extern "C" int pl_adamw_flat_planes(float* p, const float* g, float* m, float* v, int64_t n, float lr, const float* lr_dev,
                                    float beta1, float beta2, float eps, float weight_decay, int64_t t,
                                    const uint64_t* t_dev, float grad_scale, const PLAdamWPlanes* planes, void* stream) {
  if ((lr_dev != nullptr) != (t_dev != nullptr)) PL_FAIL(PL_EINVAL, "pl_adamw_flat_planes: lr_dev and t_dev go together");
  AdamWIn in = adamw_in(lr, beta1, beta2, eps, weight_decay, grad_scale, t, lr_dev, t_dev);
  if (planes && planes->nseg > 0) {
    if (planes->nseg > PL_ADAMW_MAX_SEGS || (planes->kind != 1 && planes->kind != 2) || !(planes->scale > 0.f))
      PL_FAIL(PL_EINVAL, "pl_adamw_flat_planes: bad plane description");
    if (!(aligned16(p) && aligned16(g) && aligned16(m) && aligned16(v)) || (n & 3))
      PL_FAIL(PL_EINVAL, "pl_adamw_flat_planes: arenas must be 16-byte aligned, n %% 4 == 0");
    in.nseg = planes->nseg; in.kind = planes->kind; in.pscale = planes->scale;
    for (int q = 0; q < planes->nseg; ++q) {
      const PLAdamWSeg& sg = planes->seg[q];
      if (sg.offset < 0 || sg.numel <= 0 || (sg.offset & 3) || (sg.numel & 3) || sg.offset + sg.numel > n || !sg.h ||
// ... 306 lines not shown
```

### 3d_poseestimation_amd/csrc/pl_internal.h

```cpp
#pragma once
#include <hip/hip_runtime.h>
#include <stddef.h>
#include <stdint.h>

#include "../../include/poselift.h"

namespace pl {

constexpr int kWave = 64;

void set_error(const char* fmt, ...);

#define PL_FAIL(code, ...)        \
  do {                            \
    ::pl::set_error(__VA_ARGS__); \
    return (code);                \
  } while (0)

#define PL_CHECK_LAUNCH(what)                                              \
  do {                                                                     \
    hipError_t e__ = hipGetLastError();                                    \
    if (e__ != hipSuccess)                                                 \
      PL_FAIL(PL_EHIP, "%s: launch failed: %s", what, hipGetErrorString(e__)); \
  } while (0)
// ... 88 lines not shown
int launch_bn_finalize(const float* stat, int G, int world, int B, int H,
                       const float* gamma, const float* beta, float eps, float momentum,
                       float* running_mean, float* running_var, int64_t* batches,
                       float* mean, float* rstd, float* scale, float* shift, hipStream_t s, int group_rows = 64);

struct BnFinalizeArgs {
  const float* stat;
  int G, group_rows;
  const float *gamma, *beta;
  float eps, momentum;
  float *running_mean, *running_var;
  int64_t* batches;
  float *mean, *rstd;
};
int launch_bn_apply(const float* z, const float* scale, const float* shift, const float* resid,
                    float* act, uint64_t* bits, int B, int H, float p, uint64_t seed,
                    uint64_t step, int layer, const uint64_t* inject_keep, hipStream_t s,
                    const PlaneOut* planes = nullptr, const uint64_t* step_dev = nullptr,
                    const BnFinalizeArgs* finalize = nullptr);
int mse_fwd_bwd_tick(const float* pred, const float* tgt, int64_t n, float grad_scale, float* dpred, float* loss_out,
                     void* scratch, uint64_t* tick, void* stream);

int bwd_row_chunks(int B, int H);
int launch_bn_bwd_reduce(const float* g, const uint64_t* bits, const float* z, const float* mean,
                         const float* rstd, float keep_scale, int B, int H, float* part_dy,
                         float* part_dyz, hipStream_t s, int Hc = 0, float* part_amax = nullptr, int rc = 0,
                         const float* join_g2 = nullptr, float* join_dx = nullptr);

int launch_bn_bwd_finalize(const float* part, int RC, int world, int rank, int B, int H,
                           const float* gamma, const float* rstd, float* coef, float* dgamma,
                           float* dbeta, hipStream_t s, const float* part_amax = nullptr, int n_amax = 0,
                           float* dz_scale = nullptr, int eval_mode = 0, int64_t rstride = 0, int amax_world = 1);
constexpr int kBnSmallRows = 64;
int launch_bn_small_fwd(const float* z, const float* gamma, const float* beta, float eps, float momentum, float* rm, float* rv,
                        int64_t* nbt, float* mean, float* rstd, const float* resid, float* act, uint64_t* bits, int B, int H,
                        float p, uint64_t seed, uint64_t step, int layer, const uint64_t* inject_keep, hipStream_t s,
                        const uint64_t* step_dev);
int launch_bn_small_bwd(const float* g, const uint64_t* bits, const float* z, const float* mean, const float* rstd,
                        const float* gamma, float keep_scale, int B, int H, float* dz, float* dgamma, float* dbeta, float* dbias,
                        hipStream_t s, bool tile_bits = false);
bool small_layer_ok(int B, int H, int K);
bool small_first_ok(int K);
bool small_top_ok(int O);
int launch_small_layer_fwd(const float* a, const float* W, const float* bias, const float* gamma, const float* beta, float eps,
                           float momentum, float* rm, float* rv, int64_t* nbt, float* mean, float* rstd, const float* resid,
                           float* z, float* act, uint64_t* bits, int B, int H, int K, float pdrop, uint64_t seed, uint64_t step,
                           int layer, const uint64_t* inject_keep, hipStream_t s, const uint64_t* step_dev, bool first = false,
                           const float* W2 = nullptr, float* ypart = nullptr, int O = 0,
                           const unsigned short* a_planes = nullptr, unsigned short* out_planes = nullptr);
int launch_small_layer_eval(const float* a, const float* W, const float* bias, const float* gamma, const float* beta, float eps,
                            const float* rm, const float* rv, const float* resid, float* act, int M, int H, int K, hipStream_t s,
                            bool first = false, const float* W2 = nullptr, float* ypart = nullptr, int O = 0,
                            const unsigned short* a_planes = nullptr, unsigned short* out_planes = nullptr);
int launch_small_out(const float* ypart, int NS, int M, int O, const float* bias, float* y, hipStream_t s);
int launch_small_linear_stats(const float* a, const unsigned short* a_planes, const float* W, const float* bias, float* z, int M,
                              int H, int K, float* stat_sum, float* stat_m2, int groups, hipStream_t s);
int small_mse_partials(int B, int O);
int launch_small_mse(const float* ypart, int NS, int B, int O, const float* bias, const float* tgt, float grad_scale, float* y,
                     float* dpred, float* mpart, hipStream_t s);
struct SmallBnLayer {
  const float *z, *mean, *rstd, *gamma;
  const uint64_t* bits;
  bool rowbits;
  float *dgamma, *dbeta, *dbias;
};
int launch_small_layer_bwd(const float* dz, const float* W, const float* addend, float* gout, int B, int H, int K,
                           const SmallBnLayer& below, float kscale, float* dz_lo, hipStream_t s, const float* a_in = nullptr,
                           float* dW = nullptr, const float* x1 = nullptr, float* dW1 = nullptr, int K1 = 0,
                           const struct AdamWRide* adam = nullptr);
int launch_small_top_bwd(const float* dy, const float* W2, const float* h, int B, int H, int O, float* gout, float* dW2,
                         float* db2, const SmallBnLayer& top, float kscale, float* dz_top, hipStream_t s,
                         const float* mpart = nullptr, int np = 0, float inv_n = 0.f, float* loss = nullptr,
                         uint64_t* tick = nullptr);
int launch_bn_eval_stats(const float* gamma, const float* beta, const float* rm, const float* rv, float eps, int H,
                         float* mean, float* rstd, float* scale, float* shift, hipStream_t s);
int launch_bn_bwd_dz(const float* g, const uint64_t* bits, const float* z, const float* mean,
                     const float* rstd, const float* coef, float keep_scale, int bn, int B, int H,
                     float* dz, float* part_db, hipStream_t s, int Hc = 0, const PlaneOut* planes = nullptr, int rc = 0);

int launch_reduce_slabs(const float* slabs, int nslab, int64_t n, float* out, hipStream_t s);
int launch_reduce_rows_multi(const float* const* part, const int* R, const int* H, float* const* out, int njobs,
                             hipStream_t s, const int* kind = nullptr, const int* transK = nullptr, float loss_inv_n = 0.f,
                             uint64_t* loss_tick = nullptr);
int mse_partial_only(const float* pred, const float* tgt, int64_t n, float grad_scale, float* dpred, void* scratch, void* stream);
int mse_partials(int64_t n);
bool mse_from_slabs_supported(int splits, int N);
int mse_partial_from_slabs(const float* part, int splits, int B, int N, const float* bias, const float* tgt, float grad_scale,
                           float* y, float* dpred, void* scratch, void* stream);
int launch_reduce_slabs_bias(const float* slabs, int nslab, int rows, int cols, const float* bias,
                             float* out, hipStream_t s);
int colsum_chunks(int rows);
int launch_colsum_partial(const float* X, int rows, int cols, float* part, hipStream_t s);
int launch_bn_fold_eval(const float* bias, const float* gamma, const float* beta, const float* rm,
                        const float* rv, float eps, int bn, int H, float* scale, float* shift,
                        hipStream_t s);
int launch_fill(float* p, int64_t n, float v, hipStream_t s);

bool skinny_supported(int K, int H);
int skinny_chunks(int B);
int skinny_stat_groups(int B);
int launch_skinny_wide_out(const float* X, const float* W, const float* bias, float* out, int B, int K,
                           int H, bool w_transposed, float* stat_sum, float* stat_m2, hipStream_t s,
                           const GemmArgs* bnr = nullptr);
int launch_skinny_wide_in(const float* X, const float* D, float* out, int B, int K, int H,
                          bool out_transposed, float* part, hipStream_t s, bool reduce = true, float* xsum = nullptr);
int skinny_in_chunks(int B);
bool skinny_narrow_out_supported(int H, int N);
size_t skinny_narrow_out_part_floats(int B, int H);
int launch_skinny_narrow_out(const float* h, const float* W, const float* bias, float* y, int B, int H,
                             int N, float* part, hipStream_t s, bool reduce = true);
int skinny_narrow_out_splits(int B, int H);

}
```

### 3d_poseestimation_amd/model.py

```python
import ctypes
import weakref

import torch
from torch import nn
from torch.autograd.graph import increment_version

from . import _lib
from .layout import bitmap_words_per_row, hidden_layer_prefixes, param_slots


class Linear(nn.Module):

    def __init__(self, linear_size, p_dropout=0.5, BN=True):
        super().__init__()
        self.l_size = linear_size
        self.w1 = nn.Linear(linear_size, linear_size)
        self.batch_norm1 = nn.BatchNorm1d(linear_size)
        self.w2 = nn.Linear(linear_size, linear_size)
        self.batch_norm2 = nn.BatchNorm1d(linear_size)
        self.BN = BN

    def forward(self, x):
        raise _lib.PoseliftError("residual blocks are evaluated by LinearModel.forward as one fused path")

# ... 333 lines not shown

    def workspace_view(self, ws, which, layer):
        off, size = ctypes.c_size_t(), ctypes.c_size_t()
        _lib.check(_lib.lib().pl_workspace_view(ctypes.byref(self._desc), ws["B"], which, layer,
                                                ctypes.byref(off), ctypes.byref(size)), "pl_workspace_view")
        raw = ws["buf"][off.value:off.value + size.value]
        H = self.linear_size
        if which in (0, 1):
            return raw.view(torch.float32).view(ws["B"], H)
        if which == 2:
            fmt = _lib.lib().pl_workspace_bitmap_format(ctypes.byref(self._desc), ws["B"], layer)
            _lib.check(min(fmt, 0), "pl_workspace_bitmap_format")
            words = raw.view(torch.int64)
            if fmt == 1:
                from .layout import pack_keep_bitmap, unpack_bitmap_tile
                on = unpack_bitmap_tile(words[:H].cpu().numpy().view("uint64"), ws["B"], H)
                return torch.from_numpy(pack_keep_bitmap(on).view("int64")).to(raw.device)
            return words[:ws["B"] * bitmap_words_per_row(H)].view(ws["B"], bitmap_words_per_row(H))
        return raw.view(torch.float32)

    def _run_fwd_train(self, x2, ws):
        B = x2.shape[0]
        y = torch.empty(B, self.output_size, dtype=torch.float32, device=x2.device)
        inj = self._inject_keep
        self._inject_keep = None
        if inj is not None:
            _lib.require_device_tensor(inj, "inject_keep", inj.dtype)
            want = (len(self._named_holders()), B, bitmap_words_per_row(self.linear_size))
            if tuple(inj.shape) != want or inj.element_size() != 8:
                raise _lib.PoseliftError(f"inject_keep must be 64-bit words of shape {want}")
        self._step += 1
        self._mark_wplanes()
        self._guarded(ws, lambda: _lib.lib().pl_lifter_fwd_train(
            ctypes.byref(self._desc), x2.data_ptr(), y.data_ptr(), B, ws["buf"].data_ptr(), ws["bytes"],
            self._seed, self._step, inj.data_ptr() if inj is not None else None,
            _lib.current_stream_ptr()), "pl_lifter_fwd_train")
        increment_version(self._bn_buffers)
        self.last_workspace = ws
        return y

    def _run_bwd(self, x2, gy, ws, need_dx, last_graph=True, eval_mode=False):
        B = x2.shape[0]
        accumulate = any(p.grad is not None for p in self._param_list)
        sync = self._grad_sync
        if accumulate and sync is not None and getattr(sync, "has_pending", lambda: False)():
            sync.abandon()
            raise _lib.PoseliftError(
                "gradient accumulation with overlapped all-reduce: wrap every backward but the last of an optimizer "
                "step in `with sync.no_sync():` (dp.GradSync), as with DistributedDataParallel")
        if accumulate:
            if self._flat_grad_tmp is None:
                self._flat_grad_tmp = torch.zeros_like(self._flat)
            target = self._flat_grad_tmp
        else:
            target = self.flat_grads
        dx = torch.empty_like(x2) if need_dx else None
        args = (ctypes.byref(self._desc), x2.data_ptr(), gy.data_ptr(), B, ws["buf"].data_ptr(), ws["bytes"],
                dx.data_ptr() if need_dx else None, target.data_ptr())
        if sync is not None and not accumulate and last_graph and _overlap_ok(sync) and sync.world() > 1:
            for hi, lo, a_lo, a_hi in self._bwd_ranges():
                self._guarded(ws, lambda: _lib.lib().pl_lifter_bwd_layers(*args, hi, lo, _lib.current_stream_ptr()),
                              "pl_lifter_bwd_layers")
                sync.launch_bucket(target[a_lo:a_hi])
        elif eval_mode:
            self._guarded(ws, lambda: _lib.lib().pl_lifter_bwd_eval(*args, _lib.current_stream_ptr()), "pl_lifter_bwd_eval")
        else:
            self._guarded(ws, lambda: _lib.lib().pl_lifter_bwd(*args, _lib.current_stream_ptr()), "pl_lifter_bwd")
        if accumulate:
            for s, p in zip(self._slots, self._param_list):
                gview = target[s.offset:s.offset + s.numel].view(s.shape)
                if p.grad is None:
                    p.grad = gview.clone()
                else:
                    p.grad.add_(gview)
        else:
            for s, p in zip(self._slots, self._param_list):
                if self.BN or "batch_norm" not in s.name:
                    p.grad = target[s.offset:s.offset + s.numel].view(s.shape)
        return dx

    def step_carries_adamw(self, B):
        return _lib.lib().pl_lifter_step_carries_adamw(ctypes.byref(self._desc), int(B)) == 1

    def fused_train_fwd_bwd(self, x2, target, sync=None, step_dev=None, adamw=None):
        B = x2.shape[0]
        ws = self._acquire_workspace(B)
        try:
            y = torch.empty(B, self.output_size, dtype=torch.float32, device=x2.device)
            loss = torch.empty((), dtype=torch.float32, device=x2.device)
            grads = self.flat_grads
            self._step += 1
            L = _lib.lib()
            self._desc.step_dev = step_dev.data_ptr() if step_dev is not None else None
            if adamw is not None and self.step_carries_adamw(B):
                self._desc.wplanes_valid = 0
            else:
                self._mark_wplanes()

            def call(hi, lo):
                self._guarded(ws, lambda: L.pl_lifter_train_fwd_bwd(
                    ctypes.byref(self._desc), x2.data_ptr(), target.data_ptr(), B, ws["buf"].data_ptr(), ws["bytes"],
                    self._seed, self._step, y.data_ptr(), loss.data_ptr(), grads.data_ptr(), hi, lo,
                    _lib.current_stream_ptr()), "pl_lifter_train_fwd_bwd")
            if adamw is not None:
                if sync is not None:
                    raise _lib.PoseliftError("fused_train_fwd_bwd: the in-call AdamW step and a gradient sync exclude each other")
                self._guarded(ws, lambda: L.pl_lifter_train_step(
                    ctypes.byref(self._desc), x2.data_ptr(), target.data_ptr(), B, ws["buf"].data_ptr(), ws["bytes"],
                    self._seed, self._step, y.data_ptr(), loss.data_ptr(), grads.data_ptr(), ctypes.byref(adamw),
                    _lib.current_stream_ptr()), "pl_lifter_train_step")
            elif sync is not None and sync.world() > 1 and _overlap_ok(sync):
                for hi, lo, a_lo, a_hi in self._bwd_ranges():
                    call(hi, lo)
                    sync.launch_bucket(grads[a_lo:a_hi])
            else:
                call(len(self._named_holders()), 0)
            increment_version(self._arena_tensors if adamw is not None else self._bn_buffers)
        finally:
            self._desc.step_dev = None
            self._release_workspace(ws)
        if self._param_list[-1].grad is None or self._param_list[-1].grad.data_ptr() != \
                grads.data_ptr() + 4 * self._slots[-1].offset:
            for s, p in zip(self._slots, self._param_list):
                p.grad = grads[s.offset:s.offset + s.numel].view(s.shape) if (self.BN or "batch_norm" not in s.name) else None
        self.last_workspace = ws
        return loss, y

    def forward(self, x):
        if not self._arenas_intact():
            self._flatten()
        B = x.shape[0]
        x2 = x.reshape(B, -1)
        if x2.shape[1] != self.input_size:
            raise ValueError(f"expected {self.input_size} input features, got {x2.shape[1]}")
        if x2.dtype != torch.float32:
            x2 = x2.float()
        x2 = x2.contiguous()
        _lib.require_device_tensor(x2, "x")
        _lib.require_device_tensor(self._flat, "parameters")
        if x2.device != self._flat.device:
            raise _lib.PoseliftError(f"x on {x2.device}, parameters on {self._flat.device}")
        with _lib.on_device(x2.device):
            if self.training:
                ws = self._acquire_workspace(B)
                needs_graph = torch.is_grad_enabled() and (
                    x2.requires_grad or any(p.requires_grad for p in self._param_list))
                if needs_graph:
                    return _LifterFn.apply(x2, self, ws, *self._param_list)
                try:
                    return self._run_fwd_train(x2, ws)
                finally:
                    self._release_workspace(ws)
            ws = self._acquire_workspace(B)
            if torch.is_grad_enabled() and (x2.requires_grad or any(p.requires_grad for p in self._param_list)):
                return _LifterEvalFn.apply(x2, self, ws, *self._param_list)
            try:
                y = torch.empty(B, self.output_size, dtype=torch.float32, device=x2.device)
                self._mark_wplanes()
                rc = _lib.lib().pl_lifter_fwd_eval(
                    ctypes.byref(self._desc), x2.data_ptr(), y.data_ptr(), B, ws["buf"].data_ptr(),
                    ws["bytes"], _lib.current_stream_ptr())
                _lib.check(rc, "pl_lifter_fwd_eval")
            finally:
                self._release_workspace(ws)
            return y


def weight_init(m):
    if isinstance(m, nn.Linear):
        nn.init.kaiming_normal_(m.weight)
```

### 3d_poseestimation_amd/train.py

```python
import torch
from torch.autograd.graph import increment_version

from . import _lib


class _MSEFn(torch.autograd.Function):

    @staticmethod
    def forward(ctx, pred, tgt):
        _lib.require_device_tensor(pred, "pred")
        _lib.require_device_tensor(tgt, "target")
        if pred.shape != tgt.shape:
            raise ValueError(f"MSE shapes differ: {tuple(pred.shape)} vs {tuple(tgt.shape)}")
        n = pred.numel()
        need = pred.requires_grad
        dpred = torch.empty_like(pred) if need else None
        loss = torch.empty((), dtype=torch.float32, device=pred.device)
        scratch = torch.empty(_lib.lib().pl_mse_scratch_bytes(n), dtype=torch.uint8, device=pred.device)
        with _lib.on_device(pred.device):
            rc = _lib.lib().pl_mse_fwd_bwd(pred.data_ptr(), tgt.data_ptr(), n, 1.0,
                                           dpred.data_ptr() if need else None, loss.data_ptr(),
                                           scratch.data_ptr(), _lib.current_stream_ptr())
        _lib.check(rc, "pl_mse_fwd_bwd")
        ctx.dpred = dpred
# ... 81 lines not shown
    with _lib.on_device(f.device):
        rc = _lib.lib().pl_flip_w_nhwc(f.data_ptr(), out.data_ptr(), f.shape[0], f.shape[1], f.shape[2], f.shape[3],
                                       _lib.current_stream_ptr())
    _lib.check(rc, "pl_flip_w_nhwc")
    return out


def epoch_mpjpe_mm(metric_sum, n_samples, num_of_joints=17, zero_centre=True):
    m = torch.mean((metric_sum / n_samples)[1:17])
    if num_of_joints == 17 and zero_centre:
        m = m * (17 / 16) * 1000
    return m


def _fusable(model, optimizer, y1, y2):
    from .model import LinearModel
    from .optim import FlatAdamW
    return (isinstance(model, LinearModel) and isinstance(optimizer, FlatAdamW) and optimizer._model is model
            and model.training and torch.is_grad_enabled() and not y1.requires_grad and y1.is_cuda and y2.is_cuda
            and model._inject_keep is None and model._arenas_intact()
            and y2.numel() == y2.shape[0] * model.output_size
            and y1.numel() == y1.shape[0] * model.input_size)


def train_step(model, optimizer, y1, y2, grad_sync=None):
    y1, y2 = y1.float(), y2.float()
    if _fusable(model, optimizer, y1, y2):
        with _lib.on_device(y1.device):
            x2, t2 = y1.reshape(y1.shape[0], -1).contiguous(), y2.reshape(y2.shape[0], -1).contiguous()
            if grad_sync is None and model._grad_sync is None and model.step_carries_adamw(x2.shape[0]):
                adamw = optimizer._step_struct(float(optimizer.param_groups[0]["lr"]), None, optimizer._t + 1, None)
                if adamw is not None:
                    loss, y2_hat = model.fused_train_fwd_bwd(x2, t2, None, adamw=adamw)
                    optimizer._advance_host(1)
                    return loss, y2_hat.reshape(y2.shape)
            loss, y2_hat = model.fused_train_fwd_bwd(x2, t2, grad_sync if model._grad_sync is grad_sync else None)
        optimizer.step(grad_scale=grad_sync(model) if grad_sync is not None else 1.0)
        return loss, y2_hat.reshape(y2.shape)
    optimizer.zero_grad()
    y2_hat = model(y1).reshape(y2.shape)
    loss = mse_loss(y2_hat, y2)
    loss.backward()
    if grad_sync is not None:
        optimizer.step(grad_scale=grad_sync(model))
    else:
        optimizer.step()
    return loss, y2_hat


class GraphedTrainStep:

    def __init__(self, model, optimizer, y1, y2):
        y1, y2 = y1.float(), y2.float()
        if not _fusable(model, optimizer, y1, y2) or model._grad_sync is not None:
            raise _lib.PoseliftError("GraphedTrainStep needs a training-mode LinearModel on the GPU with its FlatAdamW "
                                     "and no gradient sync attached")
        self.model, self.opt = model, optimizer
        B = y1.shape[0]
        dev = y1.device
        self._x = y1.reshape(B, -1).contiguous().clone()
        self._y = y2.reshape(B, -1).contiguous().clone()
        self._out_shape = tuple(y2.shape)
        self._tick = torch.zeros(1, dtype=torch.int64, device=dev)
        self._lr = float(optimizer.param_groups[0]["lr"])
        self._lr_dev = torch.full((1,), self._lr, dtype=torch.float32, device=dev)
        optimizer._bind()
        with _lib.on_device(dev):
            snap = [t.clone() for t in (model.flat_params, model._bn_running, model._bn_batches, optimizer._m, optimizer._v)]
            step0, t0 = model._step, optimizer._t
            train_step(model, optimizer, self._x, self._y.reshape(self._out_shape))
            for dst, src in zip((model.flat_params, model._bn_running, model._bn_batches, optimizer._m, optimizer._v), snap):
                dst.copy_(src)
            model._step, optimizer._t = step0, t0
            optimizer._step_tensor.fill_(float(t0))
            increment_version(model._arena_tensors)
            model._ensure_wplanes()
            torch.cuda.synchronize(dev)
            self.graph = torch.cuda.CUDAGraph()
            adamw = optimizer._step_struct(0.0, self._lr_dev, t0, self._tick) if model.step_carries_adamw(B) else None
            self._in_call = adamw is not None
            with torch.cuda.graph(self.graph):
                if adamw is not None:
                    self.loss, y_hat = model.fused_train_fwd_bwd(self._x, self._y, None, step_dev=self._tick, adamw=adamw)
                    self._refreshes_planes = False
                else:
                    self.loss, y_hat = model.fused_train_fwd_bwd(self._x, self._y, None, step_dev=self._tick)
                    self._refreshes_planes = optimizer._enqueue_dev(self._lr_dev, t0, self._tick)
            self.y_hat = y_hat.reshape(self._out_shape)
            model._step = step0
        self._step0, self._t0, self._seed0, self.replays = step0, t0, model._seed, 0
        self._ptrs = self._baked_ptrs()

    @property
    def inputs(self):
        return self._x, self._y

    def _baked_ptrs(self):
        return (self.model.flat_params.data_ptr(), self.opt._m.data_ptr() if self.opt._m is not None else 0,
                self.opt._v.data_ptr() if self.opt._v is not None else 0)

    def __call__(self, y1, y2):
        lr = float(self.opt.param_groups[0]["lr"])
        if lr != self._lr:
            self._lr = lr
            self._lr_dev.fill_(lr)
        ds, dt = self.model._step - self._step0, self.opt._t - self._t0
        if self.model._seed != self._seed0 or self._baked_ptrs() != self._ptrs:
            raise _lib.PoseliftError("GraphedTrainStep: the dropout seed or an arena address changed after capture "
                                     "(manual_seed, optimizer.load_state_dict, .to()): capture a new GraphedTrainStep")
        if ds != dt or ds < 0:
            raise _lib.PoseliftError(f"GraphedTrainStep: the model ran {ds} steps since capture but the optimizer {dt}: "
                                     "the graph advances both from one device counter -- capture a new one")
        if ds != self.replays:
            self._tick.fill_(ds)
            self.replays = ds
        if y1.data_ptr() != self._x.data_ptr():
            self._x.copy_(y1.reshape(self._x.shape))
        if y2.data_ptr() != self._y.data_ptr():
            self._y.copy_(y2.reshape(self._y.shape))
        if not self._in_call:
            self.model._ensure_wplanes()
        self.graph.replay()
        increment_version(self.model._arena_tensors)
        if self._refreshes_planes:
            self.model._wplanes_ver = self.model._planes_key()
        self.model._step += 1
        self.opt._advance_host(1)
        self.replays += 1
        return self.loss, self.y_hat


class GraphedModuleStep:

    def __init__(self, model, optimizer, loss_fn, inputs, target, warmup=2):
        inputs = tuple(inputs) if isinstance(inputs, (tuple, list)) else (inputs,)
        dev = target.device
        if dev.type != "cuda" or any(t.device != dev for t in inputs):
            raise _lib.PoseliftError("GraphedModuleStep: inputs and target must sit on one GPU")
        if not model.training:
            raise _lib.PoseliftError("GraphedModuleStep captures a TRAINING step: call model.train() first")
        for gr in optimizer.param_groups:
            if not gr.get("capturable", False):
                raise _lib.PoseliftError("GraphedModuleStep: the optimizer must be built with capturable=True "
                                         "(its step counter has to live on the device)")
        self.model, self.opt, self.loss_fn = model, optimizer, loss_fn
        self._state = list(model.parameters()) + list(model.buffers())
        self._in = tuple(t.detach().clone() for t in inputs)
        self._target = target.detach().clone()
        with _lib.on_device(dev):
            torch.cuda.synchronize(dev)
            state = [t for t in model.state_dict().values()]
            snap = [t.detach().clone() for t in state]
            had = {p: {k: (v.detach().clone() if torch.is_tensor(v) else v) for k, v in optimizer.state.get(p, {}).items()}
                   for gr in optimizer.param_groups for p in gr["params"]}
            side = torch.cuda.Stream(dev)
            side.wait_stream(torch.cuda.current_stream(dev))
            with torch.cuda.stream(side):
                for _ in range(max(1, int(warmup))):
                    self._step()
            torch.cuda.current_stream(dev).wait_stream(side)
            torch.cuda.synchronize(dev)
            with torch.no_grad():
                for dst, src in zip(state, snap):
                    dst.copy_(src)
                for p, old in had.items():
                    for k, v in optimizer.state.get(p, {}).items():
                        if torch.is_tensor(v):
                            v.copy_(old[k]) if k in old else v.zero_()
            optimizer.zero_grad(set_to_none=True)
            torch.cuda.synchronize(dev)
            self.graph = torch.cuda.CUDAGraph()
            with torch.cuda.graph(self.graph):
                self.loss = self._step()
        self.replays = 0

    def _step(self):
        self.opt.zero_grad(set_to_none=True)
        loss = self.loss_fn(self.model(*self._in), self._target)
        loss.backward()
        self.opt.step()
        return loss.detach()

    def __call__(self, inputs, target):
        inputs = tuple(inputs) if isinstance(inputs, (tuple, list)) else (inputs,)
        for dst, src in zip(self._in, inputs):
            dst.copy_(src)
        self._target.copy_(target)
        self.graph.replay()
        increment_version(self._state)
        self.replays += 1
        return self.loss


@torch.no_grad()
def predict_flip_tta(model, y1, out_dims=3):
    if model.training:
        raise ValueError("flip TTA is an eval-mode operation (BatchNorm on running statistics)")
    y1 = y1.float().contiguous()
    _lib.require_device_tensor(y1, "y1")
    if y1.dim() != 3 or y1.shape[1] != 17 or y1.shape[2] not in (2, 3):
        raise ValueError("flip TTA expects (B, 17, 2|3) poses")
    B, L = y1.shape[0], _lib.lib()
    xx = torch.empty((2 * B,) + tuple(y1.shape[1:]), dtype=torch.float32, device=y1.device)
# ... 55 lines not shown
```

### include/poselift.h

```cpp
#ifndef POSELIFT_H_
#define POSELIFT_H_

#include <stddef.h>
#include <stdint.h>

#ifdef __cplusplus
extern "C" {
#endif

#define PL_VERSION 111

typedef enum PLStatus {
  PL_OK = 0,
  PL_EINVAL = -1,
  PL_ESHAPE = -2,
  PL_EDTYPE = -3,
  PL_EBATCH = -4,
  PL_EHIP = -5,
  PL_EWORKSPACE = -6,
  PL_ESYNC = -7
} PLStatus;

typedef enum PLDtype { PL_F32 = 0, PL_BF16 = 1, PL_BF16X6 = 2, PL_F16X3 = 3 } PLDtype;

typedef int (*PLGatherFn)(void* user, float* buf, int64_t floats_per_rank, void* stream);
typedef struct PLSync {
  int32_t world;
  int32_t rank;
  PLGatherFn gather;
  void* user;
} PLSync;

typedef struct PLDesc {
  int32_t in_dim;
  int32_t hidden;
  int32_t out_dim;
  int32_t num_stage;
  int32_t bn;
  int32_t dtype;
  float p_dropout;
  float bn_eps;
  float bn_momentum;
  int32_t reserved;
  float* params;
  float* bn_running;
  int64_t* bn_batches;
  const PLSync* sync;
  const uint64_t* step_dev;
  void* wplanes;
  int32_t wplanes_valid;
  int32_t reserved2;
} PLDesc;

int pl_version(void);
const char* pl_last_error(void);

int64_t pl_num_hidden(const PLDesc* d);
int64_t pl_param_tensors(const PLDesc* d);
int64_t pl_param_offset(const PLDesc* d, int64_t i);
int64_t pl_param_numel(const PLDesc* d, int64_t i);
int64_t pl_param_arena_floats(const PLDesc* d);
size_t pl_workspace_bytes(const PLDesc* d, int64_t B);
int pl_workspace_view(const PLDesc* d, int64_t B, int which, int64_t layer,
                      size_t* offset_bytes, size_t* size_bytes);
int pl_workspace_bitmap_format(const PLDesc* d, int64_t B, int64_t layer);

int pl_lifter_fwd_eval(const PLDesc* d, const float* x, float* y, int64_t B,
                       void* workspace, size_t workspace_bytes, void* stream);

int pl_lifter_fwd_train(const PLDesc* d, const float* x, float* y, int64_t B,
                        void* workspace, size_t workspace_bytes,
                        uint64_t seed, uint64_t step, const uint64_t* inject_keep,
                        void* stream);

int pl_lifter_bwd(const PLDesc* d, const float* x, const float* dy, int64_t B,
                  void* workspace, size_t workspace_bytes, float* dx,
                  float* flat_grads, void* stream);

int pl_lifter_fwd_eval_saved(const PLDesc* d, const float* x, float* y, int64_t B,
                             void* workspace, size_t workspace_bytes, void* stream);
int pl_lifter_bwd_eval(const PLDesc* d, const float* x, const float* dy, int64_t B,
                       void* workspace, size_t workspace_bytes, float* dx, float* flat_grads, void* stream);

int pl_lifter_bwd_layers(const PLDesc* d, const float* x, const float* dy, int64_t B,
                         void* workspace, size_t workspace_bytes, float* dx,
                         float* flat_grads, int hi, int lo, void* stream);

int pl_lifter_train_fwd_bwd(const PLDesc* d, const float* x, const float* target, int64_t B,
                            void* workspace, size_t workspace_bytes, uint64_t seed, uint64_t step,
                            float* y, float* loss, float* flat_grads, int hi, int lo, void* stream);

typedef struct PLAdamWStep {
  float* m;
  float* v;
  float lr;
  const float* lr_dev;
  float beta1, beta2, eps, weight_decay;
  int64_t t;
  const uint64_t* t_dev;
} PLAdamWStep;
int pl_lifter_step_carries_adamw(const PLDesc* d, int64_t B);
int pl_lifter_train_step(const PLDesc* d, const float* x, const float* target, int64_t B, void* workspace,
                         size_t workspace_bytes, uint64_t seed, uint64_t step, float* y, float* loss, float* flat_grads,
                         const PLAdamWStep* opt, void* stream);

int pl_softargmax3d_nhwc_fwd(const float* logits, int64_t B, int64_t J, int64_t H, int64_t W,
                             float* coords, float* stats, void* stream);
int pl_softargmax3d_nhwc_bwd(const float* logits, const float* stats, const float* gcoords, int64_t B, int64_t J,
                             int64_t H, int64_t W, float* dlogits, void* stream);

size_t pl_conv2d_nhwc_scratch_bytes(int64_t B, int64_t H, int64_t W, int64_t Cin, int64_t Cout, int KH,
                                    int KW, int stride, int pad);
size_t pl_conv2d_nhwc_scratch_bytes_ex(int64_t B, int64_t H, int64_t W, int64_t Cin, int64_t Cout, int KH,
                                       int KW, int stride, int pad, int has_bias, int has_resid, int relu);
int pl_conv2d_nhwc_fwd(const float* x, int64_t B, int64_t H, int64_t W, int64_t Cin, const float* w,
                       int64_t Cout, int KH, int KW, int stride, int pad, const float* scale,
                       const float* shift, const float* bias, int relu, const float* resid, float* y,
                       int arith, void* scratch, size_t scratch_bytes, void* stream);

size_t pl_conv2d_nhwc_wgrad_scratch_bytes(int64_t B, int64_t H, int64_t W, int64_t Cin, int64_t Cout,
                                          int KH, int KW, int stride, int pad);
int pl_conv2d_nhwc_wgrad(const float* x, int64_t B, int64_t H, int64_t W, int64_t Cin, const float* dy,
                         int64_t Cout, int KH, int KW, int stride, int pad, float* dw, int arith, void* scratch,
                         size_t scratch_bytes, void* stream);

size_t pl_bn_train_scratch_bytes(int64_t rows, int64_t C);
int pl_bn_train_fwd(const float* z, int64_t rows, int64_t C, const float* gamma, const float* beta, float eps,
                    float momentum, float* running_mean, float* running_var, int64_t* batches, int relu,
                    float* y, uint64_t* bits, float* mean, float* rstd, void* scratch, void* stream);
int pl_bn_train_bwd(const float* dy, const uint64_t* bits, const float* z, const float* mean, const float* rstd,
                    const float* gamma, int64_t rows, int64_t C, float* dz, float* dgamma, float* dbeta,
                    void* scratch, void* stream);
int pl_add_relu_fwd(const float* a, const float* b, int64_t rows, int64_t C, float* out, uint64_t* bits, void* stream);
int pl_mask_by_bits(const float* g, const uint64_t* bits, int64_t rows, int64_t C, float* dx, void* stream);

float pl_conv_act_plane_scale(void);
int pl_planes_split(const float* x, int64_t n, int planes_mode, float scale, void* planes, void* stream);
int pl_planes_split_strided(const float* x, const int64_t* dims, const int64_t* strides, int planes_mode, float scale,
                            void* planes, void* stream);
int pl_bn_train_fwd_ex(const float* z, int64_t rows, int64_t C, const float* gamma, const float* beta, float eps,
                       float momentum, float* running_mean, float* running_var, int64_t* batches, int relu,
                       float* y, uint64_t* bits, float* mean, float* rstd, void* scratch, void* y_planes,
                       int planes_mode, const float* gemm_stat, const float* join, void* stream);
int pl_bn_train_bwd_ex(const float* dy, const uint64_t* bits, const float* z, const float* mean, const float* rstd,
                       const float* gamma, int64_t rows, int64_t C, float* dz, float* dgamma, float* dbeta,
                       void* scratch, void* dz_planes, int planes_mode, float* dz_scale, void* stream);
int pl_add_relu_fwd_ex(const float* a, const float* b, int64_t rows, int64_t C, float* out, uint64_t* bits,
                       void* out_planes, int planes_mode, void* stream);
int pl_mask_add_by_bits(const float* g, const float* g2, const uint64_t* bits, int64_t rows, int64_t C, float* dx,
                        void* stream);
int pl_bn_join_bwd(const float* g, const float* g2, const uint64_t* bits, const float* z, const float* mean,
                   const float* rstd, const float* gamma, int64_t rows, int64_t C, float* dx, float* dz, float* dgamma,
                   float* dbeta, void* scratch, void* dz_planes, int planes_mode, float* dz_scale, void* stream);

int pl_maxpool3x3s2_nhwc(const float* x, int64_t B, int64_t H, int64_t W, int64_t C, float* y, void* stream);
int pl_maxpool3x3s2_nhwc_bwd(const float* x, const float* dy, int64_t B, int64_t H, int64_t W, int64_t C,
                             float* dx, void* stream);
int pl_maxpool3x3s2_nhwc_idx(const float* x, int64_t B, int64_t H, int64_t W, int64_t C, float* y,
                             unsigned char* idx, void* stream);
int pl_maxpool3x3s2_nhwc_bwd_idx(const unsigned char* idx, const float* dy, int64_t B, int64_t H, int64_t W,
                                 int64_t C, float* dx, void* stream);
int pl_upsample2x_zero_nhwc(const float* x, int64_t B, int64_t Hi, int64_t Wi, int64_t C, float* y, void* stream);
size_t pl_colsum_scratch_bytes(int64_t rows, int64_t cols);
int pl_colsum(const float* X, int64_t rows, int64_t cols, float* out, void* scratch, void* stream);

size_t pl_deconv4x4s2_nhwc_scratch_bytes(int64_t B, int64_t Hi, int64_t Wi, int64_t Cout);
int pl_deconv4x4s2_nhwc_fwd(const float* x, int64_t B, int64_t Hi, int64_t Wi, int64_t Cin,
                            const float* w_sub, int64_t Cout, const float* scale, const float* shift,
                            int relu, float* y, int arith, void* scratch, size_t scratch_bytes, void* stream);

int pl_nhwc_to_nchw(const float* in, int64_t B, int64_t P, int64_t C, float* out, void* stream);

int pl_gather_rows2(const float* a, int64_t wa, const float* b, int64_t wb, const int64_t* idx,
                    int64_t n, int64_t table_rows, float* oa, float* ob, void* stream);

size_t pl_mse_scratch_bytes(int64_t n);
int pl_mse_fwd_bwd(const float* pred, const float* tgt, int64_t n, float grad_scale,
                   float* dpred, float* loss_out, void* scratch, void* stream);

#define PL_L1_MAX_TERMS 8
typedef struct PLL1Term {
  const float* a;
  const float* b;
  int64_t n;
// ... 164 lines not shown
```

Before: 6.938 million poses/s.

## Fuse split-K gradient reduction with AdamW and fp16 weight-plane refresh

For the large-batch planes path, the final gradient row-reduction launch now also performs the AdamW update for every parameter and writes the refreshed fp16 weight planes in the same kernel. The step counter tick moves into the MSE partial kernel so that no separate optimizer or plane-split launches are needed. This removes a separate full-arena AdamW pass and a weight-plane conversion pass, along with their extra reads of gradients and parameters. The cost is a heavier, more register-hungry reduction kernel and more complex validity checks on parameter coverage.

After: 6.924 million poses/s. About the same (-0.2%).

```diff
diff --git a/3d_poseestimation_amd/_lib.py b/3d_poseestimation_amd/_lib.py
--- a/3d_poseestimation_amd/_lib.py
+++ b/3d_poseestimation_amd/_lib.py
@@ -86,6 +86,7 @@
     "pl_lifter_train_fwd_bwd": (_c.c_int, [_D, _P, _P, _c.c_int64, _P, _c.c_size_t, _c.c_uint64, _c.c_uint64,
                                            _P, _P, _P, _c.c_int, _c.c_int, _P]),
     "pl_lifter_step_carries_adamw": (_c.c_int, [_D, _c.c_int64]),
+    "pl_lifter_step_refreshes_wplanes": (_c.c_int, [_D, _c.c_int64]),
     "pl_lifter_train_step": (_c.c_int, [_D, _P, _P, _c.c_int64, _P, _c.c_size_t, _c.c_uint64, _c.c_uint64,
                                         _P, _P, _P, _c.POINTER(PLAdamWStep), _P]),
     "pl_mse_scratch_bytes": (_c.c_size_t, [_c.c_int64]),
diff --git a/3d_poseestimation_amd/csrc/api.hip b/3d_poseestimation_amd/csrc/api.hip
--- a/3d_poseestimation_amd/csrc/api.hip
+++ b/3d_poseestimation_amd/csrc/api.hip
@@ -153,6 +153,7 @@
   bool small_layer;
   bool top_fused;
   bool adam_rides;
+  bool adam_closes;
   bool small_f16;
   bool eval_small;
   bool out_narrow;
@@ -240,6 +241,8 @@
   w.top_fused = w.small_layer && small_top_ok(d->out_dim);
   const bool small_head = w.top_fused && (d->num_stage > 0 || first_ok);
   w.adam_rides = small_head && H % 128 == 0;
+  w.adam_closes = w.planes && world == 1 && w.L > 1 && tn_splits(H, H, (int)B) == 4 && (B / 128) * (H / 128) >= 256 &&
+                  skinny_supported(d->in_dim, H) && skinny_supported(d->out_dim, H) && 3 * w.L + 3 <= kMaxStepJobs;
   w.small_f16 = d->dtype == PL_F16X3 && !w.sactp.empty() && first_ok;
   w.eval_small = d->bn && B <= kThinGemmMaxM && small_layer_ok(2, H, H) && first_ok && small_top_ok(d->out_dim);
   w.out_narrow = skinny_narrow_out_supported(H, d->out_dim);
@@ -334,6 +337,10 @@
     return reinterpret_cast<unsigned short*>(static_cast<char*>(d->wplanes) + (size_t)(l - 1) * per);
   }
   return u16(ws, w.wp[l]);
+}
+
+inline bool step_closes(const Ws& w, const PLAdamWStep* adam, bool from_output, int l_lo) {
+  return adam && w.adam_closes && from_output && l_lo == 0;
 }
 
 int split_weight_planes(const PLDesc* d, const ParamLayout& P, const Ws& w, void* ws, hipStream_t s) {
@@ -660,9 +667,12 @@
   const int64_t BH = B * H;
   const int n_amax = ((H + 255) / 256) * w.RC;
   std::vector<const float*> jpart; std::vector<float*> jout; std::vector<int> jR, jH, jkind, jtrans;
-  auto job = [&](const float* part, float* out, int R, int Hj, int kind, int transK) {
+  std::vector<unsigned short*> jplane;
+  auto job = [&](const float* part, float* out, int R, int Hj, int kind, int transK, unsigned short* plane = nullptr) {
     jpart.push_back(part); jout.push_back(out); jR.push_back(R); jH.push_back(Hj); jkind.push_back(kind); jtrans.push_back(transK);
+    jplane.push_back(plane);
   };
+  const bool adam_closes = step_closes(w, adam, do_output && l_hi == w.L - 1, l_lo) && !eval_bn && loss_out;
 
   const bool small = !eval_bn && w.bn_small, sl = !eval_bn && w.small_layer;
   auto bn_layer = [&](int l) {
@@ -771,7 +781,7 @@
                                       splits > 1 ? wsl : ly.gW, H, H, Bi, 1.0f / kActPlaneScale, dzs ? dzs + 1 : nullptr);
       tn.e.split_k = splits;
       PL_TRY(launch_gemm_planes_pair(nn, tn, s));
-      if (splits > 1) job(wsl, ly.gW, splits, H * H, 1, 0);
+      if (splits > 1) job(wsl, ly.gW, splits, H * H, 1, 0, adam_closes && d->wplanes ? wplane(d, w, ws, l) : nullptr);
     } else if (l > 0) {
       GemmArgs g = {};
       g.A = DZl; g.B = ly.W; g.M = Bi; g.N = H; g.K = H; g.lda = H; g.ldb = H; g.ldc = H; g.split_k = 1;
@@ -824,6 +834,24 @@
     inv_n = 1.0f / (float)n;
     tick = const_cast<uint64_t*>(d->step_dev);
   }
+  if (adam_closes) {
+    for (int l = 0; l < w.L; ++l) {
+      const Layer ly = layer_of(d, P, grads, l);
+      if (ly.gbeta == ly.ggamma + H) job(nullptr, ly.ggamma, 0, 2 * H, 3, 0);
+      else { job(nullptr, ly.ggamma, 0, H, 3, 0); job(nullptr, ly.gbeta, 0, H, 3, 0); }
+    }
+    int64_t covered = 0, numel = 0;
+    std::vector<StepJob> sj;
+    for (size_t k = 0; k < jpart.size(); ++k) {
+      sj.push_back(StepJob{jpart[k], jout[k], jR[k], jH[k], jkind[k], jtrans[k], jplane[k]});
+      if (jkind[k] != 2) covered += jH[k];
+    }
+    for (int64_t n : P.numel) numel += n;
+    if (covered != numel)
+      PL_FAIL(PL_EINVAL, "pl_lifter_train_step: the closing launch covers %lld of %lld parameters", (long long)covered, (long long)numel);
+    AdamWRide ar = ride(0, P.total);
+    return launch_step_tail(sj.data(), (int)sj.size(), ar, w.pkind, kWeightPlaneScale, inv_n, s);
+  }
   if (!jpart.empty())
     PL_TRY(launch_reduce_rows_multi(jpart.data(), jR.data(), jH.data(), jout.data(), (int)jpart.size(), s, jkind.data(),
                                     jtrans.data(), inv_n, tick));
@@ -1131,7 +1159,14 @@
 
 extern "C" int pl_lifter_step_carries_adamw(const PLDesc* d, int64_t B) {
   PL_TRY(check_desc(d, false));
-  return B > 0 && plan(d, B).adam_rides ? 1 : 0;
+  if (B <= 0) return 0;
+  const Ws w = plan(d, B);
+  return w.adam_rides || w.adam_closes ? 1 : 0;
+}
+
+extern "C" int pl_lifter_step_refreshes_wplanes(const PLDesc* d, int64_t B) {
+  PL_TRY(check_desc(d, false));
+  return B > 0 && d->wplanes && plan(d, B).adam_closes ? 1 : 0;
 }
 
 extern "C" int pl_lifter_train_step(const PLDesc* d, const float* x, const float* target, int64_t B, void* ws, size_t ws_bytes,
@@ -1154,9 +1189,10 @@
   PL_TRY(check_ws(w, ws, ws_bytes));
   float* dy = f32(ws, w.dyout);
   const int L = 1 + 2 * d->num_stage;
+  uint64_t* tick = step_closes(w, adam, hi == L, lo) ? const_cast<uint64_t*>(d->step_dev) : nullptr;
   if (hi == L && w.loss == Loss::PartialOnly) {
     PL_TRY(pl_lifter_fwd_train(d, x, y, B, ws, ws_bytes, seed, step, nullptr, stream));
-    PL_TRY(mse_partial_only(y, target, B * d->out_dim, 1.0f, dy, f32(ws, w.mse), stream));
+    PL_TRY(mse_partial_only(y, target, B * d->out_dim, 1.0f, dy, f32(ws, w.mse), stream, tick));
   } else if (hi == L) {
     const int H = d->hidden, O = d->out_dim;
     PL_TRY(fwd_saved_impl(d, x, y, B, ws, ws_bytes, seed, step, nullptr, stream, false, true));
@@ -1165,7 +1201,7 @@
       PL_TRY(launch_small_mse(f32(ws, w.slabs), H / 16, (int)B, O, bias, target, 1.0f, y, dy, f32(ws, w.mse), (hipStream_t)stream));
     else
       PL_TRY(mse_partial_from_slabs(f32(ws, w.slabs), skinny_narrow_out_splits((int)B, H), (int)B, O, bias, target, 1.0f, y, dy,
-                                    f32(ws, w.mse), stream));
+                                    f32(ws, w.mse), stream, tick));
   }
   return bwd_impl(d, x, dy, B, ws, ws_bytes, nullptr, grads, stream, hi == L, hi == L ? L - 1 : hi, lo, false,
                   hi == L ? loss : nullptr, w.loss == Loss::SmallMse ? small_mse_partials((int)B, d->out_dim) : 0, adam);
diff --git a/3d_poseestimation_amd/csrc/elementwise.hip b/3d_poseestimation_amd/csrc/elementwise.hip
--- a/3d_poseestimation_amd/csrc/elementwise.hip
+++ b/3d_poseestimation_amd/csrc/elementwise.hip
@@ -2,6 +2,8 @@
 #include "bn_pieces.h"
 #include "philox.h"
 #include <stdlib.h>
+
+#include <type_traits>
 
 #include "pl_internal.h"
 #include "plane_store.h"
@@ -902,10 +904,35 @@
 }
 
 constexpr int kMaxRowJobs = 16;
-struct RowJobs { const float* part[kMaxRowJobs]; float* out[kMaxRowJobs]; int R[kMaxRowJobs]; int H[kMaxRowJobs];
-                 int kind[kMaxRowJobs]; int transK[kMaxRowJobs]; float inv_n; uint64_t* tick; };
-__global__ __launch_bounds__(NTHR) void reduce_rows_multi_kernel(RowJobs j) {
-  __shared__ float red[RPARTS][RCOLS];
+template <int N>
+struct RowJobsT { const float* part[N]; float* out[N]; int R[N]; int H[N];
+                  int kind[N]; int transK[N]; float inv_n; uint64_t* tick; };
+typedef RowJobsT<kMaxRowJobs> RowJobs;
+
+struct NoTail {};
+struct StepTail {
+  AdamWRide a;
+  unsigned short* wplane[kMaxStepJobs];
+  int pkind;
+  float pscale;
+};
+
+__device__ __forceinline__ void step_adamw4(const StepTail& s, const AdamWK& k, size_t e, float4 gv, float4 pv, float4 mv,
+                                            float4 vv, unsigned short* ph, size_t r, size_t n) {
+  adamw_one(pv.x, gv.x, mv.x, vv.x, k);
+  adamw_one(pv.y, gv.y, mv.y, vv.y, k);
+  adamw_one(pv.z, gv.z, mv.z, vv.z, k);
+  adamw_one(pv.w, gv.w, mv.w, vv.w, k);
+  st4(s.a.p + e, pv); st4(s.a.m + e, mv); st4(s.a.v + e, vv);
+  if (ph) {
+    const PlaneDst d = {ph, ph + n, s.pscale, s.pkind, 0};
+    store_planes4(d, r, pv);
+  }
+}
+
+template <class Jobs, class Tail>
+__device__ __forceinline__ void reduce_rows_job(const Jobs& j, const Tail& tail, float (*red)[RCOLS]) {
+  constexpr bool kStep = std::is_same<Tail, StepTail>::value;
   const int job = blockIdx.y;
   const int R = j.R[job], H = j.H[job];
   const float* __restrict__ part = j.part[job];
@@ -920,17 +947,43 @@
     }
     return;
   }
+  if constexpr (kStep) {
+    if (j.kind[job] == 3) {
+      const int n4 = H >> 2;
+      if ((int)(blockIdx.x * NTHR) >= n4) return;
+      const AdamWK k = adamw_consts(tail.a);
+      const size_t e = (size_t)(j.out[job] - tail.a.g);
+      adamw_span(tail.a.p + e, tail.a.g + e, tail.a.m + e, tail.a.v + e, n4, blockIdx.x * NTHR + threadIdx.x,
+                 (int64_t)gridDim.x * NTHR, k);
+      return;
+    }
+  }
   if (j.kind[job] == 1) {
     const int n4 = H >> 2;
+    AdamWK k = {};
+    size_t e0 = 0;
+    unsigned short* ph = nullptr;
+    if constexpr (kStep) {
+      if ((int)(blockIdx.x * NTHR) >= n4) return;
+      k = adamw_consts(tail.a);
+      e0 = (size_t)(j.out[job] - tail.a.g);
+      ph = tail.wplane[job];
+    }
     if (R == 4) {
       for (int i = blockIdx.x * NTHR + threadIdx.x; i < n4; i += gridDim.x * NTHR) {
         const float* __restrict__ q = part + 4 * (size_t)i;
         float4 a = ld4(q);
         const float4 b1 = ld4(q + (size_t)H), b2 = ld4(q + 2 * (size_t)H), b3 = ld4(q + 3 * (size_t)H);
+        float4 pv = {}, mv = {}, vv = {};
+        if constexpr (kStep) {
+          const size_t e = e0 + 4 * (size_t)i;
+          pv = ld4(tail.a.p + e); mv = ld4(tail.a.m + e); vv = ld4(tail.a.v + e);
+        }
         a.x += b1.x; a.y += b1.y; a.z += b1.z; a.w += b1.w;
         a.x += b2.x; a.y += b2.y; a.z += b2.z; a.w += b2.w;
         a.x += b3.x; a.y += b3.y; a.z += b3.z; a.w += b3.w;
         st4(j.out[job] + 4 * (size_t)i, a);
+        if constexpr (kStep) step_adamw4(tail, k, e0 + 4 * (size_t)i, a, pv, mv, vv, ph, 4 * (size_t)i, (size_t)H);
       }
       return;
     }
@@ -941,6 +994,10 @@
         a.x += b.x; a.y += b.y; a.z += b.z; a.w += b.w;
       }
       st4(j.out[job] + 4 * (size_t)i, a);
+      if constexpr (kStep) {
+        const size_t e = e0 + 4 * (size_t)i;
+        step_adamw4(tail, k, e, a, ld4(tail.a.p + e), ld4(tail.a.m + e), ld4(tail.a.v + e), ph, 4 * (size_t)i, (size_t)H);
+      }
     }
     return;
   }
@@ -954,13 +1011,30 @@
   const float t = parts_sum(a, red, cl, p);
   if (p == 0 && c < H) {
     const int K = j.transK[job];
+    size_t at = c;
     if (K > 0) {
       const int Hc = H / K, k = c / Hc, col = c - k * Hc;
-      j.out[job][(size_t)col * K + k] = t;
-    } else {
-      j.out[job][c] = t;
-    }
-  }
+      at = (size_t)col * K + k;
+    }
+    j.out[job][at] = t;
+    if constexpr (kStep) {
+      const AdamWK k = adamw_consts(tail.a);
+      const size_t e = (size_t)(j.out[job] - tail.a.g) + at;
+      float pv = tail.a.p[e], mv = tail.a.m[e], vv = tail.a.v[e];
+      adamw_one(pv, t, mv, vv, k);
+      tail.a.p[e] = pv; tail.a.m[e] = mv; tail.a.v[e] = vv;
+    }
+  }
+}
+
+__global__ __launch_bounds__(NTHR) void reduce_rows_multi_kernel(RowJobs j) {
+  __shared__ float red[RPARTS][RCOLS];
+  reduce_rows_job(j, NoTail{}, red);
+}
+
+__global__ __launch_bounds__(NTHR) void reduce_adamw_tail_kernel(RowJobsT<kMaxStepJobs> j, StepTail tail) {
+  __shared__ float red[RPARTS][RCOLS];
+  reduce_rows_job(j, tail, red);
 }
 
 __global__ void bn_fold_eval_kernel(const float* __restrict__ bias, const float* __restrict__ gamma,
@@ -994,10 +1068,13 @@
   for (int64_t i = (int64_t)blockIdx.x * blockDim.x + threadIdx.x; i < n; i += stride) p[i] = v;
 }
 
+__device__ __forceinline__ void mse_pass_tick(uint64_t* tick) {
+  if (tick && blockIdx.x == 0 && threadIdx.x == 0) tick[0] += 1;
+}
 __global__ __launch_bounds__(NTHR) void mse_partial_kernel(const float* __restrict__ pred,
                                                            const float* __restrict__ tgt, int64_t n,
                                                            float coef, float* __restrict__ dpred,
-                                                           float* __restrict__ part) {
+                                                           float* __restrict__ part, uint64_t* tick) {
   __shared__ float sm[4];
   const int64_t stride = (int64_t)gridDim.x * blockDim.x;
   float acc = 0.f;
@@ -1008,6 +1085,7 @@
   }
   const float t = block_sum(acc, sm);
   if (threadIdx.x == 0) part[blockIdx.x] = t;
+  mse_pass_tick(tick);
 }
 
 template <int NS, int N>
@@ -1015,7 +1093,7 @@
                                                                       const float* __restrict__ bias,
                                                                       const float* __restrict__ tgt, float coef,
                                                                       float* __restrict__ y, float* __restrict__ dpred,
-                                                                      float* __restrict__ mpart) {
+                                                                      float* __restrict__ mpart, uint64_t* tick) {
   __shared__ float sm[4];
   const int64_t n = (int64_t)B * N;
   const int64_t stride = (int64_t)gridDim.x * blockDim.x;
@@ -1049,6 +1127,7 @@
   }
   const float tsum = block_sum(acc, sm);
   if (threadIdx.x == 0) mpart[blockIdx.x] = tsum;
+  mse_pass_tick(tick);
 }
 
 __global__ __launch_bounds__(NTHR) void mse_final_kernel(const float* __restrict__ part, int np,
@@ -1467,6 +1546,38 @@
   return PL_OK;
 }
 
+int launch_step_tail(const StepJob* jobs, int njobs, const AdamWRide& arenas, int pkind, float pscale, float loss_inv_n,
+                     hipStream_t s) {
+  if (njobs < 1 || njobs > kMaxStepJobs) PL_FAIL(PL_EINVAL, "step_tail: %d jobs", njobs);
+  if (!aligned16(arenas.p) || !aligned16(arenas.g) || !aligned16(arenas.m) || !aligned16(arenas.v))
+    PL_FAIL(PL_EINVAL, "step_tail: arenas must be 16-byte aligned");
+  RowJobsT<kMaxStepJobs> j = {};
+  StepTail t = {};
+  t.a = arenas; t.pkind = pkind; t.pscale = pscale;
+  j.inv_n = loss_inv_n;
+  int gx = 1;
+  for (int k = 0; k < njobs; ++k) {
+    const StepJob& q = jobs[k];
+    j.part[k] = q.part; j.out[k] = q.out; j.R[k] = q.R; j.H[k] = q.H; j.kind[k] = q.kind; j.transK[k] = q.transK;
+    t.wplane[k] = q.kind == 1 ? q.wplane : nullptr;
+    int need;
+    if (q.kind == 1 || q.kind == 3) {
+      if ((q.H & 3) || (q.kind == 1 && !aligned16(q.part)) || !aligned16(q.out) || (reinterpret_cast<uintptr_t>(q.wplane) & 7))
+        PL_FAIL(PL_EINVAL, "step_tail: job %d alignment", k);
+      need = ((q.H >> 2) + NTHR - 1) / NTHR;
+      if (need > 1024) need = 1024;
+    } else if (q.kind == 2) {
+      need = 1;
+    } else {
+      need = (q.H + RCOLS - 1) / RCOLS;
+    }
+    if (need > gx) gx = need;
+  }
+  hipLaunchKernelGGL(reduce_adamw_tail_kernel, dim3(gx, njobs), dim3(NTHR), 0, s, j, t);
+  PL_CHECK_LAUNCH("step_tail");
+  return PL_OK;
+}
+
 int colsum_chunks(int rows) {
   int rc = (rows + 63) / 64;
   if (rc > 64) rc = 64;
@@ -1530,11 +1641,11 @@
 }
 
 int pl::mse_partial_only(const float* pred, const float* tgt, int64_t n, float grad_scale, float* dpred, void* scratch,
-                         void* stream) {
+                         void* stream, uint64_t* tick) {
   if (!pred || !tgt || !scratch) PL_FAIL(PL_EINVAL, "pl_mse_fwd_bwd: null pointer");
   if (n <= 0) PL_FAIL(PL_ESHAPE, "pl_mse_fwd_bwd: n = %lld", (long long)n);
   hipLaunchKernelGGL(mse_partial_kernel, dim3(mse_blocks(n)), dim3(NTHR), 0, (hipStream_t)stream, pred, tgt, n,
-                     grad_scale * 2.0f / (float)n, dpred, (float*)scratch);
+                     grad_scale * 2.0f / (float)n, dpred, (float*)scratch, tick);
   PL_CHECK_LAUNCH("mse_partial");
   return PL_OK;
 }
@@ -1542,14 +1653,14 @@
 
 bool pl::mse_from_slabs_supported(int splits, int N) { return splits == 8 && (N == 51 || N == 34); }
 int pl::mse_partial_from_slabs(const float* part, int splits, int B, int N, const float* bias, const float* tgt, float grad_scale,
-                               float* y, float* dpred, void* scratch, void* stream) {
+                               float* y, float* dpred, void* scratch, void* stream, uint64_t* tick) {
   if (!part || !tgt || !y || !dpred || !scratch) PL_FAIL(PL_EINVAL, "mse_partial_from_slabs: null pointer");
   if (!mse_from_slabs_supported(splits, N) || B < 1) PL_FAIL(PL_ESHAPE, "mse_partial_from_slabs: splits=%d N=%d", splits, N);
   const int64_t n = (int64_t)B * N;
   const float coef = grad_scale * 2.0f / (float)n;
   const dim3 grid(mse_blocks(n)), block(NTHR);
-  if (N == 51) hipLaunchKernelGGL((mse_partial_from_slabs_kernel<8, 51>), grid, block, 0, (hipStream_t)stream, part, B, bias, tgt, coef, y, dpred, (float*)scratch);
-  else hipLaunchKernelGGL((mse_partial_from_slabs_kernel<8, 34>), grid, block, 0, (hipStream_t)stream, part, B, bias, tgt, coef, y, dpred, (float*)scratch);
+  if (N == 51) hipLaunchKernelGGL((mse_partial_from_slabs_kernel<8, 51>), grid, block, 0, (hipStream_t)stream, part, B, bias, tgt, coef, y, dpred, (float*)scratch, tick);
+  else hipLaunchKernelGGL((mse_partial_from_slabs_kernel<8, 34>), grid, block, 0, (hipStream_t)stream, part, B, bias, tgt, coef, y, dpred, (float*)scratch, tick);
   PL_CHECK_LAUNCH("mse_partial_from_slabs");
   return PL_OK;
 }
@@ -1562,7 +1673,7 @@
   const int nb = mse_blocks(n);
   const float coef = grad_scale * 2.0f / (float)n;
   hipLaunchKernelGGL(mse_partial_kernel, dim3(nb), dim3(NTHR), 0, s, pred, tgt, n, coef, dpred,
-                     (float*)scratch);
+                     (float*)scratch, (uint64_t*)nullptr);
   PL_CHECK_LAUNCH("mse_partial");
   hipLaunchKernelGGL(mse_final_kernel, dim3(1), dim3(NTHR), 0, s, (const float*)scratch, nb,
                      1.0f / (float)n, loss_out, tick);
diff --git a/3d_poseestimation_amd/csrc/pl_internal.h b/3d_poseestimation_amd/csrc/pl_internal.h
--- a/3d_poseestimation_amd/csrc/pl_internal.h
+++ b/3d_poseestimation_amd/csrc/pl_internal.h
@@ -194,11 +194,16 @@
 int launch_reduce_rows_multi(const float* const* part, const int* R, const int* H, float* const* out, int njobs,
                              hipStream_t s, const int* kind = nullptr, const int* transK = nullptr, float loss_inv_n = 0.f,
                              uint64_t* loss_tick = nullptr);
-int mse_partial_only(const float* pred, const float* tgt, int64_t n, float grad_scale, float* dpred, void* scratch, void* stream);
+constexpr int kMaxStepJobs = 32;
+struct StepJob { const float* part; float* out; int R, H, kind, transK; unsigned short* wplane; };
+int launch_step_tail(const StepJob* jobs, int njobs, const struct AdamWRide& arenas, int pkind, float pscale, float loss_inv_n,
+                     hipStream_t s);
+int mse_partial_only(const float* pred, const float* tgt, int64_t n, float grad_scale, float* dpred, void* scratch, void* stream,
+                     uint64_t* tick = nullptr);
 int mse_partials(int64_t n);
 bool mse_from_slabs_supported(int splits, int N);
 int mse_partial_from_slabs(const float* part, int splits, int B, int N, const float* bias, const float* tgt, float grad_scale,
-                           float* y, float* dpred, void* scratch, void* stream);
+                           float* y, float* dpred, void* scratch, void* stream, uint64_t* tick = nullptr);
 int launch_reduce_slabs_bias(const float* slabs, int nslab, int rows, int cols, const float* bias,
                              float* out, hipStream_t s);
 int colsum_chunks(int rows);
diff --git a/3d_poseestimation_amd/model.py b/3d_poseestimation_amd/model.py
--- a/3d_poseestimation_amd/model.py
+++ b/3d_poseestimation_amd/model.py
@@ -439,6 +439,9 @@
     def step_carries_adamw(self, B):
         return _lib.lib().pl_lifter_step_carries_adamw(ctypes.byref(self._desc), int(B)) == 1
 
+    def step_refreshes_wplanes(self, B):
+        return _lib.lib().pl_lifter_step_refreshes_wplanes(ctypes.byref(self._desc), int(B)) == 1
+
     def fused_train_fwd_bwd(self, x2, target, sync=None, step_dev=None, adamw=None):
         B = x2.shape[0]
         ws = self._acquire_workspace(B)
@@ -449,7 +452,8 @@
             self._step += 1
             L = _lib.lib()
             self._desc.step_dev = step_dev.data_ptr() if step_dev is not None else None
-            if adamw is not None and self.step_carries_adamw(B):
+            refreshes = adamw is not None and self.step_refreshes_wplanes(B)
+            if adamw is not None and self.step_carries_adamw(B) and not refreshes:
                 self._desc.wplanes_valid = 0
             else:
                 self._mark_wplanes()
@@ -473,6 +477,8 @@
             else:
                 call(len(self._named_holders()), 0)
             increment_version(self._arena_tensors if adamw is not None else self._bn_buffers)
+            if refreshes:
+                self._wplanes_ver = self._planes_key()
         finally:
             self._desc.step_dev = None
             self._release_workspace(ws)
diff --git a/3d_poseestimation_amd/train.py b/3d_poseestimation_amd/train.py
--- a/3d_poseestimation_amd/train.py
+++ b/3d_poseestimation_amd/train.py
@@ -187,7 +187,7 @@
             with torch.cuda.graph(self.graph):
                 if adamw is not None:
                     self.loss, y_hat = model.fused_train_fwd_bwd(self._x, self._y, None, step_dev=self._tick, adamw=adamw)
-                    self._refreshes_planes = False
+                    self._refreshes_planes = model.step_refreshes_wplanes(B)
                 else:
                     self.loss, y_hat = model.fused_train_fwd_bwd(self._x, self._y, None, step_dev=self._tick)
                     self._refreshes_planes = optimizer._enqueue_dev(self._lr_dev, t0, self._tick)
@@ -223,7 +223,7 @@
             self._x.copy_(y1.reshape(self._x.shape))
         if y2.data_ptr() != self._y.data_ptr():
             self._y.copy_(y2.reshape(self._y.shape))
-        if not self._in_call:
+        if self._refreshes_planes or not self._in_call:
             self.model._ensure_wplanes()
         self.graph.replay()
         increment_version(self.model._arena_tensors)
diff --git a/include/poselift.h b/include/poselift.h
--- a/include/poselift.h
+++ b/include/poselift.h
@@ -100,6 +100,7 @@
   const uint64_t* t_dev;
 } PLAdamWStep;
 int pl_lifter_step_carries_adamw(const PLDesc* d, int64_t B);
+int pl_lifter_step_refreshes_wplanes(const PLDesc* d, int64_t B);
 int pl_lifter_train_step(const PLDesc* d, const float* x, const float* target, int64_t B, void* workspace,
                          size_t workspace_bytes, uint64_t seed, uint64_t step, float* y, float* loss, float* flat_grads,
                          const PLAdamWStep* opt, void* stream);
```
